# r9y9/deepvoice3_pytorch

Measured on AMD Instinct MI355X. Metric: mel-frames/sec/node (train step, deepvoice3_ljspeech), higher is better.
Workload: dtype f16x3

## Files before the change

deepvoice3_pytorch_amd/csrc/conv_gemm_bf16x3.hip:

```cpp
#include "conv_common.h"
#include <math.h>
#include <type_traits>

typedef __bf16 bf16x8 __attribute__((ext_vector_type(8)));
typedef __bf16 bf16x2 __attribute__((ext_vector_type(2)));
typedef _Float16 f16x8 __attribute__((ext_vector_type(8)));
typedef _Float16 f16x2 __attribute__((ext_vector_type(2)));
typedef float f32x2 __attribute__((ext_vector_type(2)));

namespace {

constexpr int BKC = 32;
constexpr int KB = 4;
constexpr int HALO_MAX = 64;

__device__ __forceinline__ void split8(const float (&v)[8], bf16x8& hi, bf16x8& lo) {
#pragma unroll
  for (int i = 0; i < 8; i += 2) {
    const f32x2 f = {v[i], v[i + 1]};
    const bf16x2 h = __builtin_convertvector(f, bf16x2);
    const f32x2 r = f - __builtin_convertvector(h, f32x2);
    const bf16x2 l = __builtin_convertvector(r, bf16x2);
    hi[i] = h[0]; hi[i + 1] = h[1];
    lo[i] = l[0]; lo[i + 1] = l[1];
  }
}

template <bool F16>
__device__ __forceinline__ f32x16 mma16(const bf16x8& a, const bf16x8& b, const f32x16& c) {
  if constexpr (F16)
    return __builtin_amdgcn_mfma_f32_32x32x16_f16(__builtin_bit_cast(f16x8, a), __builtin_bit_cast(f16x8, b), c, 0, 0, 0);
  else
    return __builtin_amdgcn_mfma_f32_32x32x16_bf16(a, b, c, 0, 0, 0);
}

template <typename T>
__device__ __forceinline__ T ldg_off(const void* base, uint32_t byte_off) {
  return *reinterpret_cast<const T*>(reinterpret_cast<const char*>(base) + byte_off);
}

constexpr int STAMP_SLOTS = 192;
__device__ unsigned long long g_x3_stamps[8 * STAMP_SLOTS * 2];

template <int WM, int WN, int NI, bool MASK, int ABL = 0, int TERMS = 3, int MI = 1, bool PP = false, bool F16 = false, int DPJ = 0, int KS = 1, bool FG = false>
__global__ __launch_bounds__(WM* WN * 64 * KS) void conv_gemm_bf16x3_kernel(const ConvArgs args) {
  static_assert(!FG || (!MASK && !F16 && TERMS == 3 && ABL == 0 && DPJ == 0), "fused gate backward: the unmasked bf16-pair forms");
  static_assert(!F16 || TERMS == 3, "the fp16 form is the three-term split");
  static_assert(KS == 1 || (KS == 2 && !PP && DPJ == 0 && ABL == 0), "k-split: two groups on the in-phase loop");
  static_assert(DPJ == 0 || (DPJ == 1 || DPJ == 3), "deep prefetch: 1 or 3 taps");
  static_assert(DPJ == 0 || (!PP && MI == 1 && ABL == 0 && TERMS == 3), "deep prefetch: the in-phase three-term tiles");
  constexpr int DA = DPJ == 0 ? 1 : (DPJ == 1 ? (MASK ? 3 : 4) : 3);
  constexpr int DX = DPJ == 0 ? 1 : (DPJ == 1 ? (MASK ? 3 : 4) : 2);
  static_assert(!PP || (WM * WN == 8 && MI == 1 && (ABL == 0 || ABL >= 10)), "ping-pong: 8 waves, one row sub-tile per wave");
  constexpr int BM = WM * MI * 64, BMH = WM * MI * 32, BN = WN * NI * 32;
  constexpr int NT = WM * WN * 64;
  constexpr int AU = KB * BM / NT;
  constexpr int XI = (KB * (BN + (DPJ == 1 ? 0 : HALO_MAX)) + NT - 1) / NT;
  static_assert(KB * BM % NT == 0, "A panel must split evenly");
  const dv3_conv_desc& p = args.d;

  extern __shared__ __attribute__((aligned(16))) unsigned char smem_raw[];
  const int J = DPJ ? DPJ : p.J, dil = p.dil;
  const int BNH = BN + (J - 1) * dil;
  const int xbuf = 2 * KB * BNH;
  const int wave_all = __builtin_amdgcn_readfirstlane((int)threadIdx.x >> 6);
  const int grp = KS > 1 ? wave_all / (WM * WN) : 0;
  const int grp_units = 2 * 2 * KB * BM + 2 * xbuf;
  bf16x8* const As = reinterpret_cast<bf16x8*>(smem_raw) + grp * grp_units;
  bf16x8* const Xs = As + 2 * 2 * KB * BM;

  const int tid = (int)threadIdx.x - grp * NT;
  const int lane = tid & 63;
  const int wave = wave_all - grp * (WM * WN);
  const int wm = wave / WN, wn = wave % WN;
  const int l31 = lane & 31, lhi = lane >> 5;

  const int pid = dv3_xcd_remap(blockIdx.x, args.n_blocks);
  const int mt = pid % args.m_tiles;
  const int nt = pid / args.m_tiles;
  const int n0 = nt * BN;

  const bool gated = (p.mode == DV3_EPI_GLU || p.mode == DV3_EPI_HIGHWAY);
  int h0b, h1b, lim0, lim1;
  if (gated) {
    h0b = mt * BMH; h1b = p.a_half + mt * BMH; lim0 = p.a_half; lim1 = p.lda;
  } else {
    h0b = mt * BM; h1b = mt * BM + BMH; lim0 = lim1 = p.lda;
  }

  const int Cin = p.Cin, T = p.Tout, lda = p.lda, B = p.B;
  const int Ntot = B * T;
  const int k8_total = args.kp >> 3;
  const bf16x8* __restrict__ Wh = reinterpret_cast<const bf16x8*>(p.a_split);
  const int64_t plane = (int64_t)J * k8_total * lda;
  const uint32_t* __restrict__ xmask = p.xmask;
  const float xscale = F16 ? (float)(1 << DV3_F16_ACT_SHIFT) : 1.0f;
  const float dscale = p.drop_scale * xscale;
  const bool xpw = !MASK && !F16 && TERMS == 3 && p.x_pair != 0;

  uint32_t vbits = 0;
#pragma unroll
  for (int ni = 0; ni < NI; ++ni) {
    const int n = n0 + wn * (NI * 32) + ni * 32 + l31;
    const int bc = n / T, tc = n - bc * T;
    for (int j = 0; j < J; ++j) {
      const int ts = tc + j * dil - p.padL;
      if (n < Ntot && ts >= 0 && ts < T) vbits |= 1u << (j * NI + ni);
    }
  }
  uint32_t need = 0;
  for (int j = 0; j < J; ++j) {
    const uint32_t all = ((1u << NI) - 1u) << (j * NI);
    if (!__all((vbits & all) == all)) need |= 1u << j;
  }
  need = __builtin_amdgcn_readfirstlane(need);

  uint32_t xoff[XI];
  uint32_t xmo[MASK ? XI : 1];
  int xsh[MASK ? XI : 1];
  int xk8[XI];
  const int n_items = KB * BNH;
  const bool xbf = (TERMS == 1) && (p.io_bf16 & DV3_IO_IN_BF16);
  const uint32_t xsz = xbf ? 2u : 4u;
  const uint32_t x_rsb = (uint32_t)p.x_rs * xsz, m_rsb = (uint32_t)p.xmask_rs * 4u;
#pragma unroll
  for (int i = 0; i < XI; ++i) {
    const int idx = tid + i * NT;
    const int k8 = idx / BNH, q = idx - k8 * BNH;
    const int f = n0 - p.padL + q;
    int bf = 0, tf = 0;
    if (idx < n_items && f >= 0 && f < Ntot) {
      bf = f / T;
      tf = f - bf * T;
    }
    xk8[i] = k8 < KB ? k8 * 8 : 0;
    xoff[i] = ((uint32_t)bf * (uint32_t)p.x_bs + (uint32_t)tf) * xsz + (uint32_t)xk8[i] * x_rsb;
    if (MASK) {
      xmo[i] = ((uint32_t)(bf * Cin) * (uint32_t)p.xmask_rs + (uint32_t)(tf >> 5)) * 4u + (uint32_t)xk8[i] * m_rsb;
      xsh[i] = tf & 31;
    }
  }
  uint32_t aoff[AU];
#pragma unroll
  for (int u = 0; u < AU; ++u) {
    const int idx = tid + u * NT;
    const int col = idx % BM, k8 = idx / BM;
    const bool hi_half = col >= BMH;
    const int gcol = (hi_half ? h1b : h0b) + (col - (hi_half ? BMH : 0));
    aoff[u] = (uint32_t)(k8 * lda + (gcol < lda ? gcol : 0)) * 16u;
  }

  bf16x8 ra[DA][2][AU];
  float rx[DX][XI][8];
  uint32_t rm[MASK ? DX : 1][MASK ? XI : 1][8];

  const int nchunks_all = (Cin + BKC - 1) / BKC;
  const int nch_first = KS > 1 ? (nchunks_all + 1) / 2 : nchunks_all;
  const int c_base = grp * nch_first;
  const int nchunks = grp == 0 ? nch_first : nchunks_all - nch_first;

  auto load_A = [&](int chunk_l, int j, int slot = 0) {
    const int chunk = chunk_l + c_base;
    const bf16x8* srch = Wh + (int64_t)(j * k8_total + chunk * KB) * lda;
    const bf16x8* srcl = srch + plane;
#pragma unroll
    for (int u = 0; u < AU; ++u) {
      ra[slot][0][u] = ldg_off<bf16x8>(srch, aoff[u]);
      if (TERMS == 3) ra[slot][1][u] = ldg_off<bf16x8>(srcl, aoff[u]);
    }
  };
  auto write_A = [&](int buf, int slot = 0) {
    bf16x8* dst = As + buf * (2 * KB * BM);
#pragma unroll
    for (int u = 0; u < AU; ++u) {
      dst[tid + u * NT] = ra[slot][0][u];
      if (TERMS == 3) dst[KB * BM + tid + u * NT] = ra[slot][1][u];
    }
  };
  auto load_X = [&](int chunk_l, int slot = 0) {
    const int c0 = (chunk_l + c_base) * BKC;
    if (c0 + BKC <= Cin) {
      const char* xb = reinterpret_cast<const char*>(p.x) + (int64_t)c0 * x_rsb;
      const char* mb = reinterpret_cast<const char*>(xmask) + (int64_t)c0 * m_rsb;
      if (TERMS == 1 && xbf) {
#pragma unroll
        for (int e = 0; e < 8; ++e) {
#pragma unroll
          for (int i = 0; i < XI; ++i) {
            rx[slot][i][e] = __uint_as_float((uint32_t)ldg_off<uint16_t>(xb + (int64_t)e * x_rsb, xoff[i]) << 16);
            if (MASK) rm[slot][i][e] = ldg_off<uint32_t>(mb + (int64_t)e * m_rsb, xmo[i]);
          }
        }
      } else {
#pragma unroll
        for (int e = 0; e < 8; ++e) {
#pragma unroll
          for (int i = 0; i < XI; ++i) {
            rx[slot][i][e] = ldg_off<float>(xb + (int64_t)e * x_rsb, xoff[i]);
            if (MASK) rm[slot][i][e] = ldg_off<uint32_t>(mb + (int64_t)e * m_rsb, xmo[i]);
          }
        }
      }
    } else {
#pragma unroll
      for (int i = 0; i < XI; ++i) {
#pragma unroll
        for (int e = 0; e < 8; ++e) {
          const uint32_t dc = (uint32_t)(min(c0 + xk8[i] + e, Cin - 1) - xk8[i]);
          rx[slot][i][e] = xbf ? __uint_as_float((uint32_t)ldg_off<uint16_t>(p.x, xoff[i] + dc * x_rsb) << 16)
                         : ldg_off<float>(p.x, xoff[i] + dc * x_rsb);
          if (MASK) rm[slot][i][e] = ldg_off<uint32_t>(xmask, xmo[MASK ? i : 0] + dc * m_rsb);
        }
      }
    }
  };
  auto write_X = [&](int buf, int slot = 0) {
    bf16x8* dst = Xs + buf * xbuf;
#pragma unroll
    for (int i = 0; i < XI; ++i) {
      const int idx = tid + i * NT;
      if (idx < n_items) {
        float v[8];
#pragma unroll
        for (int e = 0; e < 8; ++e) {
          v[e] = rx[slot][i][e];
          if (MASK) v[e] *= ((rm[slot][i][e] >> xsh[i]) & 1u) ? dscale : 0.f;
          else if (F16) v[e] *= xscale;
        }
        bf16x8 hi, lo;
        if constexpr (F16) dv3_note_range(args.range_ctr, dv3_split8_f16(v, hi, lo));
        else if constexpr (!MASK && TERMS == 3) {
          if (xpw) {
            uint32_t w[8];
#pragma unroll
            for (int e = 0; e < 8; ++e) w[e] = __float_as_uint(rx[slot][i][e]);
            dv3_pair_units(w, hi, lo);
          } else split8(v, hi, lo);
        } else split8(v, hi, lo);
        dst[idx] = hi;
        if (TERMS == 3) dst[KB * BNH + idx] = lo;
      }
    }
  };

  f32x16 acc[MI][2][NI];
#pragma unroll
  for (int mi = 0; mi < MI; ++mi)
#pragma unroll
    for (int h = 0; h < 2; ++h)
#pragma unroll
      for (int ni = 0; ni < NI; ++ni)
#pragma unroll
        for (int r = 0; r < 16; ++r) acc[mi][h][ni][r] = 0.f;

  const int nsteps = (ABL == 5 || ABL == 9) ? 0 : nchunks * J;
  const int a_off = wm * (MI * 32) + l31;
  const int x_off = wn * (NI * 32) + l31;

  if constexpr (DPJ == 0) {
    load_A(0, 0);
    load_X(0);
    write_A(0);
    write_X(0);
    __syncthreads();
  }

  int n_stamp = 0;
  auto stamp = [&]() {
    if constexpr (ABL == 10) {
      if (blockIdx.x == gridDim.x / 2 && n_stamp < STAMP_SLOTS) {
        const unsigned long long t0 = __builtin_amdgcn_s_memrealtime(), t1 = __builtin_readcyclecounter();
        if (lane == 0) {
          g_x3_stamps[(wave * STAMP_SLOTS + n_stamp) * 2] = t0;
          g_x3_stamps[(wave * STAMP_SLOTS + n_stamp) * 2 + 1] = t1;
        }
      }
      ++n_stamp;
    }
  };
  int c = 0, j = 0;
  if constexpr (PP) {
    const int late = wave >> 2;
    load_A((1 < nsteps && J == 1) ? 1 : 0, (1 < nsteps && J > 1) ? 1 : 0);
    if (1 < nchunks) load_X(1);
    stamp();
    const int prio = args.prio;
    if (prio == 3 && late) __builtin_amdgcn_s_setprio(1);
    if (prio == 4 && !late) __builtin_amdgcn_s_setprio(1);
    if (late) __syncthreads();
    for (int step = 0; step < nsteps; ++step) {
      const int cur = step & 1;
      int jn = j + 1, cn = c;
      if (jn == J) { jn = 0; cn = c + 1; }
      const bool has_next = step + 1 < nsteps;
      const bool new_chunk = has_next && jn == 0;
      stamp();
      if (prio == 1) __builtin_amdgcn_s_setprio(3);
      bf16x8 ah[2][2], al[2][2], bh[2][NI], bl[2][NI];
      {
        const bf16x8* AsH = As + cur * (2 * KB * BM);
        const bf16x8* AsL = AsH + KB * BM;
        const bf16x8* XsH = Xs + (c & 1) * xbuf;
        const bf16x8* XsL = XsH + KB * BNH;
        const bool fix = (need >> j) & 1u;
        const bf16x8 zero8 = {0, 0, 0, 0, 0, 0, 0, 0};
#pragma unroll
        for (int s = 0; s < 2; ++s) {
          const int k8 = 2 * s + lhi;
          const int ai = k8 * BM + a_off;
          ah[s][0] = AsH[ai];
          ah[s][1] = AsH[ai + BMH];
          al[s][0] = (TERMS == 3) ? AsL[ai] : ah[s][0];
          al[s][1] = (TERMS == 3) ? AsL[ai + BMH] : ah[s][1];
          const int xi = k8 * BNH + x_off + j * dil;
#pragma unroll
          for (int ni = 0; ni < NI; ++ni) {
            bh[s][ni] = XsH[xi + ni * 32];
            bl[s][ni] = (TERMS == 3) ? XsL[xi + ni * 32] : bh[s][ni];
          }
        }
        if (fix) {
#pragma unroll
          for (int s = 0; s < 2; ++s)
#pragma unroll
            for (int ni = 0; ni < NI; ++ni) {
              const bool ok = (vbits >> (j * NI + ni)) & 1u;
              bh[s][ni] = ok ? bh[s][ni] : zero8;
              if (TERMS == 3) bl[s][ni] = ok ? bl[s][ni] : zero8;
            }
        }
      }
      stamp();
      write_A(cur ^ 1);
      stamp();
      if (new_chunk) {
        write_X((c + 1) & 1);
        if (cn + 1 < nchunks) load_X(cn + 1);
      }
      {
        int j2 = jn + 1, c2 = cn;
        if (j2 == J) { j2 = 0; c2 = cn + 1; }
        const bool more = step + 2 < nsteps;
        load_A(more ? c2 : c, more ? j2 : j);
      }
      stamp();
      __syncthreads();
      stamp();
      if (prio == 1) __builtin_amdgcn_s_setprio(0);
      if (prio == 2) __builtin_amdgcn_s_setprio(3);
#pragma unroll
      for (int s = 0; s < 2; ++s) {
        if (TERMS == 3) {
#pragma unroll
          for (int ni = 0; ni < NI; ++ni) {
            acc[0][0][ni] = mma16<F16>(al[s][0], bh[s][ni], acc[0][0][ni]);
            acc[0][1][ni] = mma16<F16>(al[s][1], bh[s][ni], acc[0][1][ni]);
          }
#pragma unroll
          for (int ni = 0; ni < NI; ++ni) {
            acc[0][0][ni] = mma16<F16>(ah[s][0], bl[s][ni], acc[0][0][ni]);
            acc[0][1][ni] = mma16<F16>(ah[s][1], bl[s][ni], acc[0][1][ni]);
          }
        }
#pragma unroll
        for (int ni = 0; ni < NI; ++ni) {
          acc[0][0][ni] = mma16<F16>(ah[s][0], bh[s][ni], acc[0][0][ni]);
          acc[0][1][ni] = mma16<F16>(ah[s][1], bh[s][ni], acc[0][1][ni]);
        }
      }
      stamp();
      if (prio == 2) __builtin_amdgcn_s_setprio(0);
      if (has_next || !late) __syncthreads();
      j = jn;
      c = cn;
    }
    stamp();
  } else if constexpr (DPJ > 0) {
    constexpr int U = (DPJ == 1 && DA == 4) ? 4 : 6;
    static_assert(U % DA == 0 && (U / DPJ) % DX == 0 && U % DPJ == 0 && U % 2 == 0 && (U / DPJ) % 2 == 0,
                  "ring slots and LDS buffer parities must be compile-time");
    const int last_step = nsteps - 1, last_chunk = nchunks - 1;
#pragma unroll
    for (int a = 0; a < DA; ++a)
#pragma unroll
      for (int u = 0; u < AU; ++u) ra[a][0][u] = ra[a][1][u] = bf16x8{0, 0, 0, 0, 0, 0, 0, 0};
#pragma unroll
    for (int x = 0; x < DX; ++x)
#pragma unroll
      for (int i = 0; i < XI; ++i)
#pragma unroll
        for (int e = 0; e < 8; ++e) {
          rx[x][i][e] = 0.f;
          if (MASK) rm[x][i][e] = 0u;
        }
    int s_first = -U;
    asm volatile("" : "+s"(s_first));
    for (int s0 = s_first; s0 < nsteps; s0 += U) {
#pragma unroll
      for (int dd = 0; dd < U; ++dd) {
        const int s = s0 + dd;
        const int jj = dd % DPJ;
        const int cx = dd / DPJ;
        {
          const int sa = min(max(s + DA, 0), last_step);
          load_A(sa / DPJ, sa % DPJ, dd % DA);
        }
        if (jj == 0) load_X(min(max(s0 / DPJ + cx + DX, 0), last_chunk), cx % DX);
        if (s >= 0 && s < nsteps) {
          const bf16x8* AsH = As + (dd & 1) * (2 * KB * BM);
          const bf16x8* AsL = AsH + KB * BM;
          const bf16x8* XsH = Xs + (cx & 1) * xbuf;
          const bf16x8* XsL = XsH + KB * BNH;
          const bool fix = (need >> jj) & 1u;
          const bf16x8 zero8 = {0, 0, 0, 0, 0, 0, 0, 0};
#pragma unroll
          for (int s2 = 0; s2 < 2; ++s2) {
            const int k8 = 2 * s2 + lhi;
            const int ai = k8 * BM + a_off;
            const bf16x8 ah0 = AsH[ai], ah1 = AsH[ai + BMH], al0 = AsL[ai], al1 = AsL[ai + BMH];
            bf16x8 bh[NI], bl[NI];
            const int xi = k8 * BNH + x_off + jj * dil;
#pragma unroll
            for (int ni = 0; ni < NI; ++ni) {
              bh[ni] = XsH[xi + ni * 32];
              bl[ni] = XsL[xi + ni * 32];
            }
            if (fix) {
#pragma unroll
              for (int ni = 0; ni < NI; ++ni) {
                const bool ok = (vbits >> (jj * NI + ni)) & 1u;
                bh[ni] = ok ? bh[ni] : zero8;
                bl[ni] = ok ? bl[ni] : zero8;
              }
            }
#pragma unroll
            for (int ni = 0; ni < NI; ++ni) {
              acc[0][0][ni] = mma16<F16>(al0, bh[ni], acc[0][0][ni]);
              acc[0][1][ni] = mma16<F16>(al1, bh[ni], acc[0][1][ni]);
            }
#pragma unroll
            for (int ni = 0; ni < NI; ++ni) {
              acc[0][0][ni] = mma16<F16>(ah0, bl[ni], acc[0][0][ni]);
              acc[0][1][ni] = mma16<F16>(ah1, bl[ni], acc[0][1][ni]);
            }
#pragma unroll
            for (int ni = 0; ni < NI; ++ni) {
              acc[0][0][ni] = mma16<F16>(ah0, bh[ni], acc[0][0][ni]);
              acc[0][1][ni] = mma16<F16>(ah1, bh[ni], acc[0][1][ni]);
            }
          }
        }
        write_A((dd & 1) ^ 1, (dd + 1) % DA);
        if (jj == DPJ - 1) write_X((cx & 1) ^ 1, (cx + 1) % DX);
        __syncthreads();
      }
    }
  } else
  for (int step = 0; step < (KS > 1 ? nch_first * J : nsteps); ++step) {
    if (KS > 1 && step >= nsteps) {
      __syncthreads();
      continue;
    }
    const int cur = step & 1;
    int jn = j + 1, cn = c;
    if (jn == J) { jn = 0; cn = c + 1; }
    const bool has_next = step + 1 < nsteps;
    const bool new_chunk = has_next && jn == 0;
    if (ABL != 1 && ABL != 2 && ABL != 3) {
      if (has_next) load_A(cn, jn);
      if (j == 0 && c + 1 < nchunks) load_X(c + 1);
    }

    {
      const bf16x8* AsH = As + cur * (2 * KB * BM);
      const bf16x8* AsL = AsH + KB * BM;
      const bf16x8* XsH = Xs + (c & 1) * xbuf;
      const bf16x8* XsL = XsH + KB * BNH;
      const bool fix = (need >> j) & 1u;
      const bf16x8 zero8 = {0, 0, 0, 0, 0, 0, 0, 0};
#pragma unroll
      for (int s = 0; s < 2; ++s) {
        const int k8 = 2 * s + lhi;
        const int ai = k8 * BM + a_off;
        bf16x8 ah[MI][2], al[MI][2];
#pragma unroll
        for (int mi = 0; mi < MI; ++mi) {
          ah[mi][0] = AsH[ai + mi * 32];
          ah[mi][1] = AsH[ai + mi * 32 + BMH];
          al[mi][0] = ah[mi][0];
          al[mi][1] = ah[mi][1];
          if (TERMS == 3) { al[mi][0] = AsL[ai + mi * 32]; al[mi][1] = AsL[ai + mi * 32 + BMH]; }
        }
        bf16x8 bh[NI], bl[NI];
        const int xi = k8 * BNH + x_off + j * dil;
#pragma unroll
        for (int ni = 0; ni < NI; ++ni) {
          bh[ni] = XsH[xi + ni * 32];
          bl[ni] = (TERMS == 3) ? XsL[xi + ni * 32] : bh[ni];
        }
        if (fix) {
#pragma unroll
          for (int ni = 0; ni < NI; ++ni) {
            const bool ok = (vbits >> (j * NI + ni)) & 1u;
            bh[ni] = ok ? bh[ni] : zero8;
            if (TERMS == 3) bl[ni] = ok ? bl[ni] : zero8;
          }
        }
        if (ABL == 4) {
#pragma unroll
          for (int mi = 0; mi < MI; ++mi) asm volatile("" ::"v"(ah[mi][0]), "v"(ah[mi][1]), "v"(al[mi][0]), "v"(al[mi][1]));
#pragma unroll
          for (int ni = 0; ni < NI; ++ni) asm volatile("" ::"v"(bh[ni]), "v"(bl[ni]));
          continue;
        }
        if (TERMS == 3) {
#pragma unroll
          for (int mi = 0; mi < MI; ++mi)
#pragma unroll
            for (int ni = 0; ni < NI; ++ni) {
              acc[mi][0][ni] = mma16<F16>(al[mi][0], bh[ni], acc[mi][0][ni]);
              acc[mi][1][ni] = mma16<F16>(al[mi][1], bh[ni], acc[mi][1][ni]);
            }
#pragma unroll
          for (int mi = 0; mi < MI; ++mi)
#pragma unroll
            for (int ni = 0; ni < NI; ++ni) {
              acc[mi][0][ni] = mma16<F16>(ah[mi][0], bl[ni], acc[mi][0][ni]);
              acc[mi][1][ni] = mma16<F16>(ah[mi][1], bl[ni], acc[mi][1][ni]);
            }
        }
#pragma unroll
        for (int mi = 0; mi < MI; ++mi)
#pragma unroll
          for (int ni = 0; ni < NI; ++ni) {
            acc[mi][0][ni] = mma16<F16>(ah[mi][0], bh[ni], acc[mi][0][ni]);
            acc[mi][1][ni] = mma16<F16>(ah[mi][1], bh[ni], acc[mi][1][ni]);
          }
      }
    }

    if (ABL != 2 && ABL != 3) {
      if (has_next) write_A(cur ^ 1);
      if (new_chunk) write_X((c + 1) & 1);
    }
    if (ABL != 3) __syncthreads();
    j = jn;
    c = cn;
  }

  if constexpr (KS > 1) {
    float* red = reinterpret_cast<float*>(reinterpret_cast<bf16x8*>(smem_raw) + grp_units);
    constexpr int NR = MI * 2 * NI * 16;
    static_assert((size_t)WM * WN * NR * 64 * 4 <= (size_t)(2 * 2 * KB * BM) * 16, "the accumulator image must fit one group's panels");
    float* mine = red + (wave * NR) * 64 + lane;
    if (grp == 1) {
#pragma unroll
      for (int mi = 0; mi < MI; ++mi)
#pragma unroll
        for (int h = 0; h < 2; ++h)
#pragma unroll
          for (int ni = 0; ni < NI; ++ni)
#pragma unroll
            for (int r = 0; r < 16; ++r) mine[(((mi * 2 + h) * NI + ni) * 16 + r) * 64] = acc[mi][h][ni][r];
    }
    __syncthreads();
    if (grp == 1) return;
#pragma unroll
    for (int mi = 0; mi < MI; ++mi)
#pragma unroll
      for (int h = 0; h < 2; ++h)
#pragma unroll
        for (int ni = 0; ni < NI; ++ni)
#pragma unroll
          for (int r = 0; r < 16; ++r) acc[mi][h][ni][r] += mine[(((mi * 2 + h) * NI + ni) * 16 + r) * 64];
  }
  if ((ABL != 6 && ABL != 9) || acc[0][0][0][0] + acc[MI - 1][1][0][0] + acc[0][0][NI - 1][5] + acc[MI - 1][1][NI - 1][7] == 1.2345e30f) {
    static_assert(MI == 1 || MI == 2, "row sub-tiles per wave");
    if constexpr (F16) {
      constexpr float kInv = 1.0f / (float)(1 << (DV3_F16_WEIGHT_SHIFT + DV3_F16_ACT_SHIFT));
#pragma unroll
      for (int mi = 0; mi < MI; ++mi)
#pragma unroll
        for (int h = 0; h < 2; ++h)
#pragma unroll
          for (int ni = 0; ni < NI; ++ni)
#pragma unroll
            for (int r = 0; r < 16; ++r) acc[mi][h][ni][r] *= kInv;
    }
    int n0e = n0;
    asm volatile("" : "+s"(n0e));
    int bcol[NI], tcol[NI];
    bool okc[NI];
#pragma unroll
    for (int ni = 0; ni < NI; ++ni) {
      const int n = n0e + wn * (NI * 32) + ni * 32 + l31;
      okc[ni] = n < Ntot;
      bcol[ni] = n / T;
      tcol[ni] = n - bcol[ni] * T;
    }
    if constexpr (FG) {
      const int nw0 = n0e + wn * (NI * 32);
      bool wide_done = false;
      if constexpr (NI == 2) {
        if (dv3_wide_gate_ok(p, args.wide) && (size_t)(WM * WN) * DV3_WIDE_LDS <= (size_t)(2 * 2 * KB * BM + 2 * xbuf) * 16) {
          float* wl = reinterpret_cast<float*>(smem_raw) + wave * (DV3_WIDE_LDS / 4);
#pragma unroll
          for (int mi = 0; mi < MI; ++mi) {
            const int row0 = wm * (MI * 32) + mi * 32;
            conv_epilogue_wide_block_gate<BM, BMH>(p, acc[mi][0], mt, row0, 0, lane, nw0, Ntot, wl);
            conv_epilogue_wide_block_gate<BM, BMH>(p, acc[mi][1], mt, row0, 1, lane, nw0, Ntot, wl);
          }
          wide_done = true;
        }
      }
      if (!wide_done) {
        conv_epilogue_dgrad_gate<BM, BMH, NI>(p, acc[0], mt, wm * (MI * 32), lhi, l31, bcol, tcol, okc, nw0 >> 5);
        if (MI == 2) conv_epilogue_dgrad_gate<BM, BMH, NI>(p, acc[MI - 1], mt, wm * (MI * 32) + 32, lhi, l31, bcol, tcol, okc, nw0 >> 5);
      }
    } else
    if (TERMS == 1 && (p.io_bf16 & DV3_IO_OUT_C8)) {
      conv_epilogue_c8<BM, BMH, NI>(p, acc[0], gated, mt, wm * (MI * 32), lhi, bcol, tcol, okc);
      if (MI == 2) conv_epilogue_c8<BM, BMH, NI>(p, acc[MI - 1], gated, mt, wm * (MI * 32) + 32, lhi, bcol, tcol, okc);
    } else if (NI == 2 && TERMS == 3 && ABL == 0 && dv3_wide_epilogue_ok(p, args.wide) &&
               (size_t)(WM * WN) * DV3_WIDE_LDS <= (size_t)(2 * 2 * KB * BM + 2 * xbuf) * 16) {
      if constexpr (NI == 2) {
        float* wl = reinterpret_cast<float*>(smem_raw) + wave * (DV3_WIDE_LDS / 4);
        const int nw0 = n0e + wn * (NI * 32);
#pragma unroll
        for (int mi = 0; mi < MI; ++mi) {
          const int row0 = wm * (MI * 32) + mi * 32;
          conv_epilogue_wide_block<BM, BMH>(p, acc[mi][0], mt, row0, 0, lane, nw0, Ntot, wl);
          conv_epilogue_wide_block<BM, BMH>(p, acc[mi][1], mt, row0, 1, lane, nw0, Ntot, wl);
        }
      }
    } else {
      conv_epilogue<BM, BMH, NI, ABL, TERMS == 1>(p, acc[0], gated, mt, wm * (MI * 32), lhi, bcol, tcol, okc);
      if (MI == 2)
        conv_epilogue<BM, BMH, NI, ABL, TERMS == 1>(p, acc[MI - 1], gated, mt, wm * (MI * 32) + 32, lhi, bcol, tcol, okc);
    }
  }
  stamp();
}

__global__ __launch_bounds__(256) void split_pack_kernel(const float* __restrict__ src,
                                                         bf16x8* __restrict__ dst, int J, int K,
                                                         int lda, int k8_total, int dtype, uint32_t* range_ctr) {
  const int64_t n = (int64_t)J * k8_total * lda;
  const int64_t idx = (int64_t)blockIdx.x * 256 + threadIdx.x;
  if (idx >= n) return;
  const int m = (int)(idx % lda);
  const int64_t row = idx / lda;
  const int j = (int)(row / k8_total), k8 = (int)(row % k8_total);
  float v[8];
#pragma unroll
  for (int i = 0; i < 8; ++i) {
    const int k = k8 * 8 + i;
    v[i] = (k < K) ? src[((int64_t)j * K + k) * lda + m] : 0.f;
    if (dtype == DV3_SPLIT_DTYPE_F16) v[i] *= (float)(1 << DV3_F16_WEIGHT_SHIFT);
  }
  bf16x8 hi, lo;
  if (dtype == DV3_SPLIT_DTYPE_F16) dv3_note_range(range_ctr, dv3_split8_f16(v, hi, lo)); else split8(v, hi, lo);
  dst[idx] = hi;
  dst[n + idx] = lo;
}

#ifdef DV3_X3_ISA_ONLY
#ifndef DV3_X3_ISA_KS
#define DV3_X3_ISA_KS 1
#endif
template __global__ void conv_gemm_bf16x3_kernel<2, 2, 1, DV3_X3_ISA_MASK, 0, 3, 1, false, DV3_X3_ISA_F16, DV3_X3_ISA_DPJ, DV3_X3_ISA_KS>(const ConvArgs);
}
#else
template <int WM, int WN, int NI, bool MASK, int TERMS, int MI = 1, bool PP = false, bool F16 = false, int DPJ = 0, int KS = 1, bool FG = false>
int launch_x3_m(const ConvArgs& a, size_t lds, hipStream_t st) {
  static bool attr_set = false;
  if (!attr_set) {
    hipError_t e = hipFuncSetAttribute((const void*)conv_gemm_bf16x3_kernel<WM, WN, NI, MASK, 0, TERMS, MI, PP, F16, DPJ, KS, FG>,
                                       hipFuncAttributeMaxDynamicSharedMemorySize, 160 * 1024);
    if (e != hipSuccess) {
      dv3_set_error("conv_gemm_bf16x3: hipFuncSetAttribute: %s", hipGetErrorString(e));
      return DV3_ELAUNCH;
    }
    attr_set = true;
  }
  dim3 grid(a.n_blocks), block(WM * WN * 64 * KS);
  hipLaunchKernelGGL((conv_gemm_bf16x3_kernel<WM, WN, NI, MASK, 0, TERMS, MI, PP, F16, DPJ, KS, FG>), grid, block, lds * KS, st, a);
  return dv3_check_launch("conv_gemm_bf16x3");
}
int g_x3_ablate = 0;
#ifdef DV3_EXPERIMENTS
template <int ABL>
int launch_x3_abl(const ConvArgs& a, size_t lds, hipStream_t st) {
  (void)hipFuncSetAttribute((const void*)conv_gemm_bf16x3_kernel<2, 2, 2, false, ABL>,
                      hipFuncAttributeMaxDynamicSharedMemorySize, 160 * 1024);
  hipLaunchKernelGGL((conv_gemm_bf16x3_kernel<2, 2, 2, false, ABL>), dim3(a.n_blocks), dim3(256), lds, st, a);
  return dv3_check_launch("conv_gemm_bf16x3(abl)");
}
#endif
int g_x3_pingpong = 1;
template <int WM, int WN, int NI, int MI, bool PP>
int launch_x3_big_pp(const ConvArgs& a, size_t lds, hipStream_t st) {
  if (a.d.split_terms == DV3_SPLIT_F16X3)
    return a.d.xmask ? launch_x3_m<WM, WN, NI, true, 3, MI, PP, true>(a, lds, st) : launch_x3_m<WM, WN, NI, false, 3, MI, PP, true>(a, lds, st);
  if (a.d.split_terms == 1)
    return a.d.xmask ? launch_x3_m<WM, WN, NI, true, 1, MI, PP>(a, lds, st) : launch_x3_m<WM, WN, NI, false, 1, MI, PP>(a, lds, st);
  return a.d.xmask ? launch_x3_m<WM, WN, NI, true, 3, MI, PP>(a, lds, st) : launch_x3_m<WM, WN, NI, false, 3, MI, PP>(a, lds, st);
}
template <int WM, int WN, int NI, int MI>
int launch_x3_big(const ConvArgs& a, size_t lds, hipStream_t st) {
#ifdef DV3_EXPERIMENTS
  if constexpr (WM == 2 && WN == 4 && MI == 1) {
    if (g_x3_ablate == 10 && g_x3_pingpong && !a.d.xmask && (a.d.split_terms == 0 || a.d.split_terms == 3)) {
      (void)hipFuncSetAttribute((const void*)conv_gemm_bf16x3_kernel<2, 4, 2, false, 10, 3, 1, true>,
                                hipFuncAttributeMaxDynamicSharedMemorySize, 160 * 1024);
      hipLaunchKernelGGL((conv_gemm_bf16x3_kernel<2, 4, 2, false, 10, 3, 1, true>), dim3(a.n_blocks), dim3(512), lds, st, a);
      return dv3_check_launch("conv_gemm_bf16x3(stamps)");
    }
  }
#endif
  if constexpr (WM * WN == 8 && MI == 1) {
    if (g_x3_pingpong) return launch_x3_big_pp<WM, WN, NI, MI, true>(a, lds, st);
  }
  return launch_x3_big_pp<WM, WN, NI, MI, false>(a, lds, st);
}
template <int WM, int WN, int NI>
int launch_x3(const ConvArgs& a, size_t lds, hipStream_t st) {
#ifdef DV3_EXPERIMENTS
  if (g_x3_ablate && WM == 2 && WN == 2 && NI == 2 && !a.d.xmask && (a.d.split_terms == 0 || a.d.split_terms == 3)) {
    switch (g_x3_ablate) {
      case 1: return launch_x3_abl<1>(a, lds, st);
      case 2: return launch_x3_abl<2>(a, lds, st);
      case 3: return launch_x3_abl<3>(a, lds, st);
      case 4: return launch_x3_abl<4>(a, lds, st);
      case 5: return launch_x3_abl<5>(a, lds, st);
      case 6: return launch_x3_abl<6>(a, lds, st);
      case 7: return launch_x3_abl<7>(a, lds, st);
      case 8: return launch_x3_abl<8>(a, lds, st);
      case 9: return launch_x3_abl<9>(a, lds, st);
    }
  }
#endif
  if constexpr (WM == 2 && WN == 2 && NI == 1) {
    if (a.ks == 2 && a.d.split_terms != 1) {
      const bool f16 = a.d.split_terms == DV3_SPLIT_F16X3, m = a.d.xmask != nullptr;
      if (f16) return m ? launch_x3_m<2, 2, 1, true, 3, 1, false, true, 0, 2>(a, lds, st) : launch_x3_m<2, 2, 1, false, 3, 1, false, true, 0, 2>(a, lds, st);
      return m ? launch_x3_m<2, 2, 1, true, 3, 1, false, false, 0, 2>(a, lds, st) : launch_x3_m<2, 2, 1, false, 3, 1, false, false, 0, 2>(a, lds, st);
    }
  }
#ifdef DV3_EXPERIMENTS
  if constexpr (WM == 2 && WN == 2 && NI == 1) {
    if (a.dp == 1 || a.dp == 3) {
      const bool f16 = a.d.split_terms == DV3_SPLIT_F16X3, m = a.d.xmask != nullptr;
      if (a.dp == 1) {
        if (f16) return m ? launch_x3_m<2, 2, 1, true, 3, 1, false, true, 1>(a, lds, st) : launch_x3_m<2, 2, 1, false, 3, 1, false, true, 1>(a, lds, st);
        return m ? launch_x3_m<2, 2, 1, true, 3, 1, false, false, 1>(a, lds, st) : launch_x3_m<2, 2, 1, false, 3, 1, false, false, 1>(a, lds, st);
      }
      if (f16) return m ? launch_x3_m<2, 2, 1, true, 3, 1, false, true, 3>(a, lds, st) : launch_x3_m<2, 2, 1, false, 3, 1, false, true, 3>(a, lds, st);
      return m ? launch_x3_m<2, 2, 1, true, 3, 1, false, false, 3>(a, lds, st) : launch_x3_m<2, 2, 1, false, 3, 1, false, false, 3>(a, lds, st);
    }
  }
#endif
  if (a.d.split_terms == DV3_SPLIT_F16X3)
    return a.d.xmask ? launch_x3_m<WM, WN, NI, true, 3, 1, false, true>(a, lds, st) : launch_x3_m<WM, WN, NI, false, 3, 1, false, true>(a, lds, st);
  if (a.d.split_terms == 1)
    return a.d.xmask ? launch_x3_m<WM, WN, NI, true, 1>(a, lds, st) : launch_x3_m<WM, WN, NI, false, 1>(a, lds, st);
  return a.d.xmask ? launch_x3_m<WM, WN, NI, true, 3>(a, lds, st) : launch_x3_m<WM, WN, NI, false, 3>(a, lds, st);
}

int g_x3_ks = 1;
int g_x3_ks_max_blocks = 256, g_x3_ks_min_steps = 8;
int g_x3_dp = 0;
int g_x3_rel8 = 86;
int g_x3_j1_flat = 1;
int g_x3_rel2 = 112;
const TileCfg* pick_tile_x3(const dv3_conv_desc* d, bool gated, int want_tile) {
  const TileCfg* best = nullptr;
  double best_cost = 0;
  const int64_t ntot = (int64_t)d->B * d->Tout;
  for (const TileCfg& c : kCfgs) {
    if (want_tile && c.id != want_tile) continue;
    if (d->pg && !(c.id == 1 || c.id == 2 || c.id == 8 || c.id == 9)) continue;
    const int BM = c.wm * c.mi * 64, BMH = c.wm * c.mi * 32, BN = c.wn * c.ni * 32;
    const int64_t mt = gated ? dv3_cdiv(d->Cg, BMH) : dv3_cdiv(d->M, BM);
    const int64_t ntl = dv3_cdiv64(ntot, BN);
    const double slots = c.id > 6 ? 256.0 : 512.0;
    const double blocks = (double)mt * ntl;
    const double full = floor(blocks / slots), rem = blocks - slots * full;
    const double rounds = (full + (rem == 0 ? 0.0 : (c.id <= 6 && rem <= 256 ? 0.6 : 1.0))) * (slots / 512.0);
    static const double kRel[10] = {0, 1.0, 1.12, 2.0, 2.2, 1.8, 2.0, 9.9, 0.93, 0.87};
    double rel = c.id == 2 ? g_x3_rel2 * 0.01 : c.id == 8 ? g_x3_rel8 * 0.01 : kRel[c.id];
    if (g_x3_j1_flat && d->J == 1 && d->Cin <= 512 && (c.id == 1 || c.id == 2 || c.id == 8 || c.id == 9)) rel = 1.0;
    const double cost = rounds * BM * BN * rel;
    if (!best || cost < best_cost) {
      best = &c;
      best_cost = cost;
    }
  }
  return best;
}

}

int g_x3_pp2 = 128;
extern int g_pp2_ord, g_pp2_ord_u, g_pp2_ord_m, g_pp2_abl, g_pp2_sk, g_pp2_sk_overhead, g_pp2_sk_gain, g_pp2_sk_abl, g_pp2_fast_tail;
int g_x3_pp2_sk_units = 8;
int dv3_conv_gemm_pp2_dispatch(const dv3_conv_desc* d, hipStream_t st);
int g_x3_wide = 1;
int g_x3_prio = 0;

int dv3_conv_gemm_bf16x3_dispatch(const dv3_conv_desc* d, hipStream_t st) {
  const bool gated = d->mode == DV3_EPI_GLU || d->mode == DV3_EPI_HIGHWAY;
  if (d->a_bs != 0 || (d->lda & 3) || d->Tin != d->Tout) return 1;
  if ((d->J - 1) * d->dil > HALO_MAX || d->J * 2 > 32) return 1;
  if ((int64_t)d->B * d->Tout >= (1ll << 30) || (int64_t)d->B * d->x_bs >= (1ll << 30)) return 1;
  if (d->xmask && (int64_t)d->B * d->Cin * d->xmask_rs >= (1ll << 30)) return 1;
  if ((int64_t)d->J * ((d->Cin + 31) / 32 * 4) * d->lda >= (1ll << 27)) return 1;
  const bool gated0 = d->mode == DV3_EPI_GLU || d->mode == DV3_EPI_HIGHWAY;
  const int64_t pp2_tiles = (int64_t)(gated0 ? dv3_cdiv(d->Cg, 128) : dv3_cdiv(d->M, 256)) * dv3_cdiv64((int64_t)d->B * d->Tout, 256);
  const bool sk_fill = d->sk_ws && g_pp2_sk && (d->mode != DV3_EPI_DGRAD || g_pp2_sk >= 2) && g_x3_pp2 > 0 && pp2_tiles * (d->Cin / 32) >= (int64_t)g_x3_pp2_sk_units * 256;
  if (d->tile_hint == 30 || (g_x3_pp2 > 0 && d->tile_hint == 0 && (pp2_tiles >= g_x3_pp2 || sk_fill))) {
    const int rc = dv3_conv_gemm_pp2_dispatch(d, st);
    if (rc != 1) return rc;
    if (d->tile_hint == 30) return 1;
  }
  const TileCfg* best = pick_tile_x3(d, gated, d->tile_hint > 20 ? d->tile_hint - 20 : 0);
  if (!best) return 1;
  bool ks_ok = false;
  if (g_x3_ks && d->split_terms != 1 && (d->tile_hint == 0 || d->tile_hint == 22)) {
    const int64_t nb2 = (int64_t)(gated ? dv3_cdiv(d->Cg, 64) : dv3_cdiv(d->M, 128)) * dv3_cdiv64((int64_t)d->B * d->Tout, 64);
    const int nch = (d->Cin + 31) / 32;
    const int ksteps = nch * d->J;
    ks_ok = nch >= 2 && (g_x3_ks == 2 || (ksteps >= g_x3_ks_min_steps && nb2 <= (ksteps >= 16 ? g_x3_ks_max_blocks : g_x3_ks_max_blocks * 5 / 8)));
    if (ks_ok && d->tile_hint == 0 && (best->id == 4 || best->id == 6)) best = &kCfgs[1];
  }
  const int BM = best->wm * best->mi * 64, BMH = best->wm * best->mi * 32, BN = best->wn * best->ni * 32;
  const int BNH = BN + (d->J - 1) * d->dil;
  const size_t lds = (size_t)(2 * 2 * KB * BM + 2 * 2 * KB * BNH) * 16;
  if (lds > 160 * 1024) return 1;
  ConvArgs a;
  a.d = *d;
  a.a_scalar = 0;
  a.wide = g_x3_wide;
  a.prio = g_x3_prio;
  a.range_ctr = d->split_terms == DV3_SPLIT_F16X3 ? dv3_range_ctr() : nullptr;
  a.kp = (d->Cin + 31) / 32 * 32;
  a.m_tiles = gated ? dv3_cdiv(d->Cg, BMH) : dv3_cdiv(d->M, BM);
  a.n_tiles = (int)dv3_cdiv64((int64_t)d->B * d->Tout, BN);
  const int64_t nb = (int64_t)a.m_tiles * a.n_tiles;
  DV3_REQUIRE(nb < (1ll << 31), "conv_gemm: grid too large");
  a.n_blocks = (int)nb;
  a.ks = (ks_ok && best->id == 2 && 2 * lds <= 160 * 1024) ? 2 : 0;
  a.dp = 0;
#ifdef DV3_EXPERIMENTS
  if (best->id == 2 && d->split_terms != 1 && (d->J == 1 || d->J == 3) && g_x3_dp) {
    if (g_x3_dp == 2 || nb <= 2 * 256) a.dp = d->J;
  }
#endif
  g_dv3_last_conv = (d->split_terms == 1 ? 4000 : d->split_terms == DV3_SPLIT_F16X3 ? 5000 : 3000) + best->id * 10 +
                    ((best->id >= 8 && g_x3_pingpong) ? 1 : 0) + (a.dp ? 5 : 0) + (a.ks == 2 ? 2 : 0);
  if (d->pg) {
    if (d->xmask || d->split_terms == DV3_SPLIT_F16X3 || d->split_terms == 1) return 1;
    g_dv3_last_conv += 600;
    switch (best->id) {
      case 1: return launch_x3_m<2, 2, 2, false, 3, 1, false, false, 0, 1, true>(a, lds, st);
      case 2: return a.ks == 2 ? launch_x3_m<2, 2, 1, false, 3, 1, false, false, 0, 2, true>(a, lds, st)
                               : launch_x3_m<2, 2, 1, false, 3, 1, false, false, 0, 1, true>(a, lds, st);
      case 8: return launch_x3_m<4, 2, 2, false, 3, 1, true, false, 0, 1, true>(a, lds, st);
      case 9: return launch_x3_m<2, 4, 2, false, 3, 1, true, false, 0, 1, true>(a, lds, st);
    }
    return 1;
  }
  switch (best->id) {
    case 1: return launch_x3<2, 2, 2>(a, lds, st);
    case 2: return launch_x3<2, 2, 1>(a, lds, st);
    case 3: return launch_x3<4, 1, 1>(a, lds, st);
    case 4: return launch_x3<2, 1, 1>(a, lds, st);
    case 5: return launch_x3<1, 2, 2>(a, lds, st);
    case 6: return launch_x3<1, 2, 1>(a, lds, st);
    case 7: return launch_x3_big<2, 2, 2, 2>(a, lds, st);
    case 8: return launch_x3_big<4, 2, 2, 1>(a, lds, st);
    case 9: return launch_x3_big<2, 4, 2, 1>(a, lds, st);
  }
  return 1;
}

extern int g_wgrad_tile, g_wgrad_prio, g_wgrad_t2_abl, g_wgrad_taps2_default, g_wgrad_t2_window, g_wgrad_t2_il;
extern int g_spk_prefetch;
extern int g_gate_c8_fast;
extern int g_loss_fast_log;
extern int g_gate_vec;
extern int g_wn_bwd_vec4;
extern int g_wgrad_c8_pf2, g_wgrad_c8_il, g_wgrad_c8_tr, g_spk_abl;
int dv3_planes_debug_set(int what, int value);
int dv3_c8pp_debug_set(int what, int value);
int dv3_conv_census_set(int on);
extern "C" int dv3_debug_set(int what, int value) {
#ifndef DV3_EXPERIMENTS
  DV3_REQUIRE(!(value != 0 && (what == 1 || what == 6 || what == 13 || what == 16 || what == 21 || what == 26 || what == 28 || what == 32 || what == 43)),
              "debug_set(%d, %d): ablation variants are not in this build (make EXP=1)", what, value);
#endif
  if (what >= 4 && what <= 8) return dv3_planes_debug_set(what, value);
  if (what == 40) return dv3_conv_census_set(value);
  if (what == 19 || what == 21 || what == 30 || what == 32 || (what >= 34 && what <= 36)) return dv3_c8pp_debug_set(what, value);
  if (what == 20) g_wgrad_c8_pf2 = value;
  if (what == 49) g_wgrad_c8_il = value;
  if (what == 9) g_x3_rel2 = value;
  if (what == 12) g_x3_pp2 = value;
  if (what == 13) g_pp2_abl = value;
  if (what == 29 || what == 31) {
    const bool ship = value == 0 || value == 17 || value == 81;
#ifndef DV3_EXPERIMENTS
    DV3_REQUIRE(ship, "debug_set(%d, %d): this LOAD-phase variant is not in this build (make EXP=1)", what, value);
#endif
    if (what == 29) { g_pp2_ord_u = ship ? value : 0; g_pp2_ord = ship ? 0 : value; }
    else g_pp2_ord_m = ship ? value : 0;
  }
  if (what == 50) g_pp2_fast_tail = value;
  if (what == 51) g_wn_bwd_vec4 = value;
  if (what == 52) g_wgrad_c8_tr = value;
  if (what == 54) g_spk_prefetch = value;
  if (what == 55) g_gate_vec = value;
  if (what == 56) g_gate_c8_fast = value;
  if (what == 57) g_loss_fast_log = value;
  if (what == 22) g_pp2_sk = value;
  if (what == 23) g_pp2_sk_overhead = value;
  if (what == 24) g_pp2_sk_gain = value;
  if (what == 25) g_x3_pp2_sk_units = value;
  if (what == 26) g_pp2_sk_abl = value;
  if (what == 27) g_x3_j1_flat = value;
  if (what == 43) g_x3_dp = value;
  if (what == 42) g_x3_rel8 = value;
  if (what == 44) g_x3_ks = value;
  if (what == 45) g_x3_ks_max_blocks = value;
  if (what == 46) g_x3_ks_min_steps = value;
  if (what == 28) g_spk_abl = value;
  if (what == 14) g_x3_prio = value;
  if (what == 18) g_x3_wide = value;
  if (what == 15) g_wgrad_prio = value;
  if (what == 16) g_wgrad_t2_abl = value;
  if (what == 17) g_wgrad_taps2_default = value;
  if (what == 47) g_wgrad_t2_window = value;
  if (what == 48) g_wgrad_t2_il = value;
  if (what == 1) g_x3_ablate = value;
  if (what == 2) g_wgrad_tile = value;
  if (what == 3) g_x3_pingpong = value;
  return DV3_OK;
}

int dv3_pp2_read_stamps(void* dst, int64_t bytes);
int dv3_decode_read_stamps(void* dst, int64_t bytes);
int dv3_conv_census_read(int what, void* dst, int64_t bytes);
extern "C" int dv3_debug_read(int what, void* dst, int64_t bytes) {
  if (what == 40 || what == 41) return dv3_conv_census_read(what, dst, bytes);
  if (what == 2 && dst) return dv3_pp2_read_stamps(dst, bytes);
  if (what == 3 && dst) return dv3_decode_read_stamps(dst, bytes);
  DV3_REQUIRE(what == 1 && dst && bytes > 0 && bytes <= (int64_t)sizeof(unsigned long long) * 8 * STAMP_SLOTS * 2,
              "debug_read: bad arguments");
  hipError_t e = hipMemcpyFromSymbol(dst, HIP_SYMBOL(g_x3_stamps), (size_t)bytes, 0, hipMemcpyDeviceToHost);
  if (e != hipSuccess) {
    dv3_set_error("debug_read: %s", hipGetErrorString(e));
    return DV3_ELAUNCH;
  }
  return DV3_OK;
}

extern "C" int dv3_split_pack_bf16(const float* packed, uint16_t* out, int32_t J, int32_t K,
                                   int32_t lda, int32_t dtype, void* stream) {
  DV3_REQUIRE(dtype == DV3_SPLIT_DTYPE_BF16 || dtype == DV3_SPLIT_DTYPE_F16, "split_pack: bad dtype");
  DV3_REQUIRE(packed && out, "split_pack: null pointer");
  DV3_REQUIRE(J >= 1 && K >= 1 && lda >= 1 && ((uintptr_t)out & 15) == 0, "split_pack: bad arguments");
  const int k8_total = (K + 31) / 32 * 4;
  const int64_t n = (int64_t)J * k8_total * lda;
  hipLaunchKernelGGL(split_pack_kernel, dim3((unsigned)dv3_cdiv64(n, 256)), dim3(256), 0,
                     (hipStream_t)stream, packed, reinterpret_cast<bf16x8*>(out), J, K, lda, k8_total, (int)dtype,
                     dv3_range_ctr());
  return dv3_check_launch("split_pack_bf16");
}
#endif
```

deepvoice3_pytorch_amd/csrc/conv_gemm_pp2.hip:

```cpp
#include "conv_common.h"
#include <math.h>
#include <type_traits>

typedef __bf16 bf16x8 __attribute__((ext_vector_type(8)));
typedef __bf16 bf16x2 __attribute__((ext_vector_type(2)));
typedef _Float16 f16x8 __attribute__((ext_vector_type(8)));
typedef float f32x2 __attribute__((ext_vector_type(2)));

namespace {

constexpr int BKC = 32, KB = 4, HALO_MAX = 64;
constexpr int BM = 256, BMH = 128, BN = 256, NT = 512, MI = 2, NI = 2, WN = 4;
constexpr int JT = 3;
constexpr int AU = KB * BM / NT;
constexpr int XI = (KB * (BN + HALO_MAX) + NT - 1) / NT;
static_assert(AU == 2, "one panel unit per k16 phase");

__device__ __forceinline__ void pp2_split8(const float (&v)[8], bf16x8& hi, bf16x8& lo) {
#pragma unroll
  for (int i = 0; i < 8; i += 2) {
    const f32x2 f = {v[i], v[i + 1]};
    const bf16x2 h = __builtin_convertvector(f, bf16x2);
    const f32x2 r = f - __builtin_convertvector(h, f32x2);
    const bf16x2 l = __builtin_convertvector(r, bf16x2);
    hi[i] = h[0]; hi[i + 1] = h[1];
    lo[i] = l[0]; lo[i + 1] = l[1];
  }
}
template <bool F16>
__device__ __forceinline__ f32x16 pp2_mma(const bf16x8& a, const bf16x8& b, const f32x16& c) {
  if constexpr (F16)
    return __builtin_amdgcn_mfma_f32_32x32x16_f16(__builtin_bit_cast(f16x8, a), __builtin_bit_cast(f16x8, b), c, 0, 0, 0);
  else
    return __builtin_amdgcn_mfma_f32_32x32x16_bf16(a, b, c, 0, 0, 0);
}
template <bool OPAQUE>
__device__ __forceinline__ const ConvArgs* dv3_opaque_args(const ConvArgs* a) {
  if constexpr (OPAQUE) {
    int off = 0;
    asm volatile("" : "+s"(off));
    return reinterpret_cast<const ConvArgs*>(reinterpret_cast<const char*>(a) + off);
  } else {
    return a;
  }
}
template <typename T>
__device__ __forceinline__ T pp2_ldg(const void* base, uint32_t byte_off) {
  return *reinterpret_cast<const T*>(reinterpret_cast<const char*>(base) + byte_off);
}

constexpr int PP2_STAMPS = 320;
__device__ unsigned long long g_pp2_stamps[8 * PP2_STAMPS * 2];

template <bool MASK, bool F16, int ABL = 0, bool SK = false, int ORD = 0, bool PW = false, bool FG = false>
__global__ __launch_bounds__(NT) void conv_gemm_pp2_kernel(const ConvArgs args) {
  static_assert(!PW || (!MASK && !F16 && !SK), "pair words: the unmasked bf16-pair tile-per-workgroup form");
  static_assert(!FG || (!MASK && !F16 && !SK), "fused gate backward: the unmasked bf16-pair tile-per-workgroup form");
  const dv3_conv_desc& p = args.d;
  int n_stamp = 0;
  auto stamp = [&]() {
    if constexpr (ABL == 4) {
      if (blockIdx.x == gridDim.x / 2 + 3 && n_stamp < PP2_STAMPS) {
        const unsigned long long t0 = __builtin_amdgcn_s_memrealtime(), t1 = __builtin_readcyclecounter();
        if ((threadIdx.x & 63) == 0) {
          g_pp2_stamps[((threadIdx.x >> 6) * PP2_STAMPS + n_stamp) * 2] = t0;
          g_pp2_stamps[((threadIdx.x >> 6) * PP2_STAMPS + n_stamp) * 2 + 1] = t1;
        }
      }
      ++n_stamp;
    }
  };
  stamp();
  extern __shared__ __attribute__((aligned(16))) unsigned char smem_raw[];
  constexpr int J = JT;
  bf16x8* const As = reinterpret_cast<bf16x8*>(smem_raw);
  bf16x8* const Xs = As + 2 * 2 * KB * BM;

  int pid_ = dv3_xcd_remap(blockIdx.x, args.n_blocks);
  if constexpr (SK) {
    const int q = 1 << args.sk_qshift;
    pid_ = (pid_ & ~(q - 1)) + (q - 1 - (pid_ & (q - 1)));
  }
  const int pid = pid_;
  const int nchunks = p.Cin / BKC;
  int seg_u = 0, seg_end = 0, sk_base = 0, sk_rem = 0, sk_g0 = 0;
  if constexpr (SK) {
    const int grp = pid >> args.sk_qshift, slot = pid & ((1 << args.sk_qshift) - 1);
    const bool big = grp < args.sk_tr;
    sk_base = big ? args.sk_base : args.sk_base2;
    sk_rem = big ? args.sk_rem : args.sk_rem2;
    sk_g0 = (grp * args.sk_tg + min(grp, args.sk_tr)) << args.sk_shift;
    seg_u = sk_g0 + slot * sk_base + min(slot, sk_rem);
    seg_end = seg_u + sk_base + (slot < sk_rem ? 1 : 0);
  }
  constexpr bool DMA_A = ABL == 11;
  constexpr bool WIDE_GLU = (ORD & 32) != 0;
  int tid_ = threadIdx.x;
  const int wave_s = __builtin_amdgcn_readfirstlane(tid_ >> 6);
  do {
  const ConvArgs& A = *dv3_opaque_args<SK>(&args);
  const dv3_conv_desc& p = A.d;
  const int dil = p.dil;
  const int BNH = BN + (J - 1) * dil;
  const int xbuf = 2 * KB * BNH;
  if constexpr (SK) {
    int lane_;
    asm volatile("v_mbcnt_lo_u32_b32 %0, -1, 0\n\tv_mbcnt_hi_u32_b32 %0, -1, %0" : "=v"(lane_));
    tid_ = wave_s * 64 + lane_;
  }
  const int tid = tid_;
  const int lane = tid & 63;
  const int wave = __builtin_amdgcn_readfirstlane(tid >> 6);
  const int wm = wave / WN, wn = wave % WN;
  const int l31 = lane & 31, lhi = lane >> 5;
  int tile_ = pid, c0_ = 0, c1_ = nchunks;
  if constexpr (SK) {
    tile_ = seg_u >> A.sk_shift;
    c0_ = seg_u - tile_ * nchunks;
    c1_ = min(nchunks, c0_ + (seg_end - seg_u));
  }
  const int tile = tile_, c0 = SK ? c0_ : 0, c1 = SK ? c1_ : nchunks;
  const int mt = SK ? (tile & (A.m_tiles - 1)) : tile % A.m_tiles;
  const int nt = SK ? (tile >> A.sk_mshift) : tile / A.m_tiles;
  const int n0 = nt * BN;

  const bool gated = (p.mode == DV3_EPI_GLU || p.mode == DV3_EPI_HIGHWAY);
  int h0b, h1b;
  if (gated) {
    h0b = mt * BMH; h1b = p.a_half + mt * BMH;
  } else {
    h0b = mt * BM; h1b = mt * BM + BMH;
  }

  const int Cin = p.Cin, T = p.Tout, lda = p.lda, B = p.B;
  const int Ntot = B * T;
  const int k8_total = A.kp >> 3;
  const bf16x8* __restrict__ Wh = reinterpret_cast<const bf16x8*>(p.a_split);
  const int64_t plane = (int64_t)J * k8_total * lda;
  const float xscale = F16 ? (float)(1 << DV3_F16_ACT_SHIFT) : 1.0f;
  const float dscale = p.drop_scale * xscale;

  uint32_t vbits = 0;
#pragma unroll
  for (int ni = 0; ni < NI; ++ni) {
    const int n = n0 + wn * (NI * 32) + ni * 32 + l31;
    const int bc = n / T, tc = n - bc * T;
    for (int j = 0; j < J; ++j) {
      const int ts = tc + j * dil - p.padL;
      if (n < Ntot && ts >= 0 && ts < T) vbits |= 1u << (j * NI + ni);
    }
  }
  uint32_t need = 0;
  for (int j = 0; j < J; ++j) {
    const uint32_t all = ((1u << NI) - 1u) << (j * NI);
    if (!__all((vbits & all) == all)) need |= 1u << j;
  }
  need = __builtin_amdgcn_readfirstlane(need);

  uint32_t xoff[XI];
  const int n_items = KB * BNH;
  const uint32_t x_rsb = (uint32_t)p.x_rs * 4u;
  const uint32_t c8p = (uint32_t)((Cin + 31) / 32 * 4);
#pragma unroll
  for (int i = 0; i < XI; ++i) {
    const int idx = tid + i * NT;
    const int k8 = idx / BNH, q = idx - k8 * BNH;
    const int f = n0 - p.padL + q;
    int bf = 0, tf = 0;
    if (idx < n_items && f >= 0 && f < Ntot) {
      bf = f / T;
      tf = f - bf * T;
    }
    const int xk8 = k8 < KB ? k8 * 8 : 0;
    xoff[i] = ((uint32_t)bf * (uint32_t)p.x_bs + (uint32_t)tf) * 4u + (uint32_t)xk8 * x_rsb;
  }
  constexpr bool LEAN = (ORD & 2) != 0 && !SK;
  uint32_t aoff_r[2] = {0u, 0u};
  auto aoff_of = [&](int u) -> uint32_t {
    if constexpr (LEAN) return aoff_r[u];
    int t_ = tid;
    asm volatile("" : "+v"(t_));
    const int idx = t_ + u * NT;
    const int col = idx % BM, k8 = idx / BM;
    const bool hi_half = col >= BMH;
    const int gcol = (hi_half ? h1b : h0b) + (col - (hi_half ? BMH : 0));
    return (uint32_t)(k8 * lda + (gcol < lda ? gcol : 0)) * 16u;
  };

  if constexpr (LEAN) {
#pragma unroll
    for (int u = 0; u < 2; ++u) {
      const int idx = tid + u * NT;
      const int col = idx % BM, k8 = idx / BM;
      const bool hi_half = col >= BMH;
      const int gcol = (hi_half ? h1b : h0b) + (col - (hi_half ? BMH : 0));
      aoff_r[u] = (uint32_t)(k8 * lda + (gcol < lda ? gcol : 0)) * 16u;
    }
  }

  bf16x8 ra[2];
  float rx[XI][8];
  uint32_t rk[MASK ? XI : 1];

  auto load_A_unit = [&](int chunk, int j, auto uc) {
    constexpr int u = decltype(uc)::value;
    const bf16x8* srch = Wh + (int64_t)(j * k8_total + chunk * KB) * lda;
    const uint32_t ao = aoff_of(u);
    ra[0] = pp2_ldg<bf16x8>(srch, ao);
    ra[1] = pp2_ldg<bf16x8>(srch + plane, ao);
  };
  auto write_A_unit = [&](int buf, auto uc) {
    constexpr int u = decltype(uc)::value;
    bf16x8* dst = As + buf * (2 * KB * BM);
    dst[tid + u * NT] = ra[0];
    dst[KB * BM + tid + u * NT] = ra[1];
  };
  auto dma_A_unit = [&](int buf, int chunk, int j, auto uc) {
    constexpr int u = decltype(uc)::value;
    const bf16x8* srch = Wh + (int64_t)(j * k8_total + chunk * KB) * lda;
    const uint32_t ao = aoff_of(u);
    bf16x8* dst = As + buf * (2 * KB * BM) + u * NT + wave * 64;
    typedef const __attribute__((address_space(1))) void* gptr;
    typedef __attribute__((address_space(3))) void* lptr;
    __builtin_amdgcn_global_load_lds((gptr)(reinterpret_cast<const char*>(srch) + ao), (lptr)dst, 16, 0, 0);
    __builtin_amdgcn_global_load_lds((gptr)(reinterpret_cast<const char*>(srch + plane) + ao), (lptr)(dst + KB * BM), 16, 0, 0);
  };
  auto load_X_half = [&](int chunk, auto ic, auto hc) {
    constexpr int i = decltype(ic)::value, h = decltype(hc)::value;
    const char* xb = reinterpret_cast<const char*>(p.x) + (int64_t)(chunk * BKC) * x_rsb;
    uint32_t rs = x_rsb;
    asm volatile("" : "+s"(rs));
#pragma unroll
    for (int e = 4 * h; e < 4 * h + 4; ++e) {
      uint32_t er = (uint32_t)e * rs;
      if constexpr (SK) {
        if (e == 0) { er = 0; asm volatile("" : "+s"(er)); }
      }
      rx[i][e] = pp2_ldg<float>(xb, xoff[i] + er);
    }
    if constexpr (MASK && h == 1) {
      int t_ = tid;
      asm volatile("" : "+v"(t_));
      const int idx = t_ + i * NT;
      const int k8 = idx / BNH, q = idx - k8 * BNH;
      const int f = n0 - p.padL + q;
      int bf = 0, tf = 0;
      if (idx < n_items && f >= 0 && f < Ntot) {
        bf = f / T;
        tf = f - bf * T;
      }
      const uint32_t mo = ((uint32_t)bf * c8p + (uint32_t)(k8 < KB ? k8 : 0)) * (uint32_t)T + (uint32_t)tf;
      rk[i] = (uint32_t)pp2_ldg<uint8_t>(p.xmask_c8 + (int64_t)chunk * 4 * T, mo);
    }
  };
  auto write_X_item = [&](int buf, auto ic) {
    constexpr int i = decltype(ic)::value;
    bf16x8* dst = Xs + buf * xbuf;
    const int idx = tid + i * NT;
    float v[8];
    uint32_t keep = MASK ? rk[i] : 0u;
    if constexpr (MASK && SK) asm("" : "+v"(keep));
#pragma unroll
    for (int e = 0; e < 8; ++e) {
      v[e] = rx[i][e];
      if constexpr (MASK) v[e] *= ((keep >> e) & 1u) ? dscale : 0.f;
      else if (F16) v[e] *= xscale;
    }
    bf16x8 hi, lo;
    if constexpr (PW) {
      uint32_t w[8];
#pragma unroll
      for (int e = 0; e < 8; ++e) w[e] = __float_as_uint(rx[i][e]);
      dv3_pair_units(w, hi, lo);
    } else if constexpr (F16 && LEAN) {
      const float m0 = fmaxf(fmaxf(fabsf(v[0]), fabsf(v[1])), fabsf(v[2]));
      const float m1 = fmaxf(fmaxf(fabsf(v[3]), fabsf(v[4])), fabsf(v[5]));
      const float m = fmaxf(fmaxf(m0, m1), fmaxf(fabsf(v[6]), fabsf(v[7])));
      const bool bad = !(m <= 65504.f);
      if (__builtin_expect(__any(bad), 0)) {
        dv3_note_range(A.range_ctr, dv3_split8_f16(v, hi, lo));
      } else {
        f16x8 h8, l8;
#pragma unroll
        for (int e = 0; e < 8; e += 2) {
          const f32x2 f = {v[e], v[e + 1]};
          typedef _Float16 f16x2_ __attribute__((ext_vector_type(2)));
          const f16x2_ h = __builtin_convertvector(f, f16x2_);
          h8[e] = h[0]; h8[e + 1] = h[1];
          if constexpr ((ORD & 8) != 0) {
            uint32_t l2 = 0u;
            const uint32_t h2 = __builtin_bit_cast(uint32_t, h);
            asm("v_fma_mixlo_f16 %0, %1, -1.0, %2 op_sel:[0,0,0] op_sel_hi:[1,0,0]" : "+v"(l2) : "v"(h2), "v"(v[e]));
            asm("v_fma_mixhi_f16 %0, %1, -1.0, %2 op_sel:[1,0,0] op_sel_hi:[1,0,0]" : "+v"(l2) : "v"(h2), "v"(v[e + 1]));
            const f16x2_ l = __builtin_bit_cast(f16x2_, l2);
            l8[e] = l[0]; l8[e + 1] = l[1];
          } else {
            l8[e] = (_Float16)(v[e] - (float)h[0]);
            l8[e + 1] = (_Float16)(v[e + 1] - (float)h[1]);
          }
        }
        hi = __builtin_bit_cast(bf16x8, h8);
        lo = __builtin_bit_cast(bf16x8, l8);
      }
    } else if constexpr (F16) dv3_note_range(A.range_ctr, dv3_split8_f16(v, hi, lo)); else pp2_split8(v, hi, lo);
    if (idx < n_items) {
      dst[idx] = hi;
      dst[KB * BNH + idx] = lo;
    }
  };
  uint32_t sbad = 0;
  auto write_X_item_nb = [&](int buf, auto ic) {
    constexpr int i = decltype(ic)::value;
    bf16x8* dst = Xs + buf * xbuf;
    const int idx = tid + i * NT;
    float v[8];
    const uint32_t keep = MASK ? rk[i] : 0u;
#pragma unroll
    for (int e = 0; e < 8; ++e) {
      v[e] = rx[i][e];
      if constexpr (MASK) {
        v[e] *= ((keep >> e) & 1u) ? dscale : 0.f;
        asm("" : "+v"(v[e]));
      } else if (F16) v[e] *= xscale;
    }
    bf16x8 hi, lo;
    if constexpr (PW) {
      uint32_t w[8];
#pragma unroll
      for (int e = 0; e < 8; ++e) w[e] = __float_as_uint(rx[i][e]);
      dv3_pair_units(w, hi, lo);
    } else if constexpr (F16) {
      const bool bad = dv3_split8_f16(v, hi, lo);
      sbad += (uint32_t)__builtin_popcountll(__ballot(bad));
    } else {
      pp2_split8(v, hi, lo);
    }
    const int spare = 2 * xbuf - buf * xbuf;
    const bool live = i < 2 || idx < n_items;
    dst[live ? idx : spare] = hi;
    dst[live ? KB * BNH + idx : spare + 1] = lo;
  };
  using U0 = std::integral_constant<int, 0>;
  using U1 = std::integral_constant<int, 1>;
  using U2 = std::integral_constant<int, 2>;
  constexpr bool CVC = (ORD & 64) != 0 && !SK;
  static_assert(XI == 3 && JT == 3, "three activation items per thread, one per tap's pair of k16 phases");

  f32x16 acc[MI][2][NI];
  float zero_ = 0.f;
  if constexpr (SK) asm volatile("" : "+v"(zero_));
#pragma unroll
  for (int mi = 0; mi < MI; ++mi)
#pragma unroll
    for (int h = 0; h < 2; ++h)
#pragma unroll
      for (int ni = 0; ni < NI; ++ni)
#pragma unroll
        for (int r = 0; r < 16; ++r) acc[mi][h][ni][r] = zero_;

  const int a_off = wm * (MI * 32) + l31;
  const int x_off = wn * (NI * 32) + l31;

  load_A_unit(c0, 0, U0{});
  write_A_unit(0, U0{});
  load_A_unit(c0, 0, U1{});
  load_X_half(c0, U0{}, U0{}); load_X_half(c0, U0{}, U1{});
  load_X_half(c0, U1{}, U0{}); load_X_half(c0, U1{}, U1{});
  load_X_half(c0, U2{}, U0{}); load_X_half(c0, U2{}, U1{});
  write_A_unit(0, U1{});
  write_X_item(0, U0{});
  write_X_item(0, U1{});
  write_X_item(0, U2{});
  __syncthreads();
  {
    const int cp = min(c0 + 1, c1 - 1);
    if (!DMA_A) load_A_unit(c0, 1, U0{});
    load_X_half(cp, U0{}, U0{});
    load_X_half(cp, U0{}, U1{});
    load_X_half(cp, U1{}, U0{}); load_X_half(cp, U1{}, U1{});
    load_X_half(cp, U2{}, U0{});
    if constexpr (!CVC) load_X_half(cp, U2{}, U1{});
  }

  const bool pf_on = (ORD & 4) != 0 && !SK && gated && p.r != nullptr;
  const int late = wave >> 2;
  stamp();
  if (late) __syncthreads();
  for (int c = c0; c < c1; ++c) {
    const int cr = c - c0;
    const bf16x8* XsH = Xs + (cr & 1) * xbuf;
    const bf16x8* XsL = XsH + KB * BNH;
    const int cx = min(c + 2, c1 - 1);
    const bool last_chunk = c + 1 == c1;
#pragma unroll
    for (int q = 0; q < 2 * JT; ++q) {
      constexpr int dummy = 0; (void)dummy;
      const int j = q >> 1, s = q & 1;
      const int cur = (cr * JT + j) & 1;
      const bf16x8* AsH = As + cur * (2 * KB * BM);
      const bf16x8* AsL = AsH + KB * BM;
      const bool fix = (need >> j) & 1u;
      stamp();
      bf16x8 ah[MI][2], al[MI][2], bh[NI], bl[NI];
      auto read_frags = [&](bool do_a, bool do_b) {
        const int k8 = 2 * s + lhi;
        if (do_a) {
          const int ai = k8 * BM + a_off;
#pragma unroll
          for (int mi = 0; mi < MI; ++mi) {
            ah[mi][0] = AsH[ai + mi * 32];
            ah[mi][1] = AsH[ai + mi * 32 + BMH];
            al[mi][0] = AsL[ai + mi * 32];
            al[mi][1] = AsL[ai + mi * 32 + BMH];
          }
        }
        if (do_b) {
          const int xi = k8 * BNH + x_off + j * dil;
#pragma unroll
          for (int ni = 0; ni < NI; ++ni) {
            bh[ni] = XsH[xi + ni * 32];
            bl[ni] = XsL[xi + ni * 32];
          }
        }
      };
      auto fix_frags = [&]() {
        const int k8 = 2 * s + lhi; (void)k8;
        if (fix) {
          const bf16x8 zero8 = {0, 0, 0, 0, 0, 0, 0, 0};
#pragma unroll
          for (int ni = 0; ni < NI; ++ni) {
            const bool ok = (vbits >> (j * NI + ni)) & 1u;
            bh[ni] = ok ? bh[ni] : zero8;
            bl[ni] = ok ? bl[ni] : zero8;
          }
        }
      };
      if constexpr ((ORD & 1) != 0) {
        read_frags(true, (ORD & 16) == 0);
        __builtin_amdgcn_sched_barrier(0);
      }
      if (ABL != 2) {
        int jn = j + 1, cn = c;
        if (jn >= JT) { jn = 0; cn = c + 1; }
        int j2 = jn + 1, c2 = cn;
        if (j2 >= JT) { j2 = 0; c2 = cn + 1; }
        if (cn >= c1) { cn = c; jn = j; }
        if (c2 >= c1) { c2 = c; j2 = j; }
        if constexpr (DMA_A) {
          if (s == 0) {
            dma_A_unit(cur ^ 1, cn, jn, U0{});
            dma_A_unit(cur ^ 1, cn, jn, U1{});
          }
          (void)c2; (void)j2;
        } else if (s == 0) {
          if (ABL != 9) write_A_unit(cur ^ 1, U0{});
          if (ABL != 7) load_A_unit(cn, jn, U1{});
        } else {
          if (ABL != 9) write_A_unit(cur ^ 1, U1{});
          if (ABL != 7) load_A_unit(c2, j2, U0{});
        }
        constexpr bool WX = ABL != 8, LX = ABL != 6;
        if constexpr (CVC) {
          const int cx1 = min(c + 1, c1 - 1);
          if (q == 0) load_X_half(cx1, U2{}, U1{});
          if (q == 1) load_X_half(cx, U0{}, U0{});
          if (q == 2) load_X_half(cx, U0{}, U1{});
          if (q == 3) load_X_half(cx, U1{}, U0{});
          if (q == 4) load_X_half(cx, U1{}, U1{});
          if (q == 5) load_X_half(cx, U2{}, U0{});
        } else {
        if (q == 0) { if (WX) write_X_item((cr + 1) & 1, U0{}); if (LX) load_X_half(cx, U0{}, U0{}); }
        if (q == 1) { if (LX) load_X_half(cx, U0{}, U1{}); }
        if (q == 2) { if (WX) write_X_item((cr + 1) & 1, U1{}); if (LX) load_X_half(cx, U1{}, U0{}); }
        if (q == 3) { if (LX) load_X_half(cx, U1{}, U1{}); }
        if (q == 4) { if (WX) write_X_item((cr + 1) & 1, U2{}); if (LX) load_X_half(cx, U2{}, U0{}); }
        if (q == 5) { if (LX) load_X_half(cx, U2{}, U1{}); }
        }
        if constexpr ((ORD & 4) != 0 && !SK) {
          if ((q == 1 || q == 3) && last_chunk && pf_on) {
            typedef const __attribute__((address_space(1))) void* gptr;
            typedef __attribute__((address_space(3))) void* lptr;
            unsigned char* strip = smem_raw + (size_t)(2 * 2 * KB * BM + 2 * xbuf) * 16 + wave * 256;
            int t_ = tid;
            asm volatile("" : "+v"(t_));
            const int row = t_ >> 2, col = (t_ & 3) * 64 + (q >> 1) * 32;
            const int ch = min(mt * BMH + row, p.Cg - 1);
            const int n = min(n0 + col, Ntot - 1);
            const int bb = n / T, tt = n - bb * T;
            const uint32_t po = ((uint32_t)bb * (uint32_t)p.r_bs + (uint32_t)ch * (uint32_t)p.r_rs + (uint32_t)tt) * 4u;
            __builtin_amdgcn_global_load_lds((gptr)(reinterpret_cast<const char*>(p.r) + po), (lptr)strip, 4, 0, 0);
          }
        }
      }
      __builtin_amdgcn_sched_barrier(0);
      stamp();
      if constexpr ((ORD & 1) == 0) read_frags(true, true);
      else if constexpr ((ORD & 16) != 0) read_frags(false, true);
      fix_frags();
      if constexpr (ABL == 4) {
        asm volatile("s_waitcnt lgkmcnt(0)" ::: "memory");
        stamp();
      }
      __syncthreads();
      if (ABL != 5) __builtin_amdgcn_sched_barrier(0);
      stamp();
      if (ABL != 1) {
#pragma unroll
        for (int mi = 0; mi < MI; ++mi)
#pragma unroll
          for (int ni = 0; ni < NI; ++ni) {
            acc[mi][0][ni] = pp2_mma<F16>(al[mi][0], bh[ni], acc[mi][0][ni]);
            acc[mi][1][ni] = pp2_mma<F16>(al[mi][1], bh[ni], acc[mi][1][ni]);
          }
#pragma unroll
        for (int mi = 0; mi < MI; ++mi)
#pragma unroll
          for (int ni = 0; ni < NI; ++ni) {
            acc[mi][0][ni] = pp2_mma<F16>(ah[mi][0], bl[ni], acc[mi][0][ni]);
            acc[mi][1][ni] = pp2_mma<F16>(ah[mi][1], bl[ni], acc[mi][1][ni]);
          }
#pragma unroll
        for (int mi = 0; mi < MI; ++mi)
#pragma unroll
          for (int ni = 0; ni < NI; ++ni) {
            acc[mi][0][ni] = pp2_mma<F16>(ah[mi][0], bh[ni], acc[mi][0][ni]);
            acc[mi][1][ni] = pp2_mma<F16>(ah[mi][1], bh[ni], acc[mi][1][ni]);
          }
      } else {
#pragma unroll
        for (int mi = 0; mi < MI; ++mi) asm volatile("" ::"v"(ah[mi][0]), "v"(ah[mi][1]), "v"(al[mi][0]), "v"(al[mi][1]));
#pragma unroll
        for (int ni = 0; ni < NI; ++ni) asm volatile("" ::"v"(bh[ni]), "v"(bl[ni]));
      }
      if constexpr (CVC) {
        if (q == 0) write_X_item_nb((cr + 1) & 1, U0{});
        if (q == 2) write_X_item_nb((cr + 1) & 1, U1{});
        if (q == 4) write_X_item_nb((cr + 1) & 1, U2{});
        if ((q & 1) == 0) {
#pragma unroll
          for (int m = 0; m < 22; ++m) {
            __builtin_amdgcn_sched_group_barrier(0x008, 1, 0);
            __builtin_amdgcn_sched_group_barrier(0x002, 3, 0);
          }
          __builtin_amdgcn_sched_group_barrier(0x008, 1, 0);
          __builtin_amdgcn_sched_group_barrier(0x200, 1, 0);
          __builtin_amdgcn_sched_group_barrier(0x008, 1, 0);
          __builtin_amdgcn_sched_group_barrier(0x200, 1, 0);
        }
      }
      stamp();
      if (ABL != 5) __builtin_amdgcn_sched_barrier(0);
      if (!(last_chunk && q == 2 * JT - 1) || !late) __syncthreads();
    }
  }
  stamp();
  if constexpr (CVC && F16) {
    if (sbad != 0 && lane == 0 && A.range_ctr) atomicAdd(A.range_ctr, sbad);
  }

  bool run_tail = true;
  if constexpr (SK) {
    constexpr int ACC = MI * 2 * NI * 16;
#ifdef DV3_EXPERIMENTS
    const int sk_abl = A.sk_abl;
#else
    constexpr int sk_abl = 0;
#endif
    float* const ws = A.sk_ws;
    int* const flags = A.sk_flags;
    if (c0 != 0) {
      char* dst = reinterpret_cast<char*>(ws) + ((size_t)pid * (ACC * NT) + (size_t)tid * 4) * 4;
      if (!(sk_abl & 1))
#pragma unroll
      for (int mi = 0; mi < MI; ++mi)
#pragma unroll
        for (int h = 0; h < 2; ++h)
#pragma unroll
          for (int ni = 0; ni < NI; ++ni)
#pragma unroll
            for (int r4 = 0; r4 < 4; ++r4) {
              typedef float f32x4_ __attribute__((ext_vector_type(4)));
              const f32x4_ v4 = {acc[mi][h][ni][r4 * 4], acc[mi][h][ni][r4 * 4 + 1], acc[mi][h][ni][r4 * 4 + 2], acc[mi][h][ni][r4 * 4 + 3]};
              const char* d4 = dst + (size_t)((((mi * 2 + h) * NI + ni) * 4 + r4) * NT) * 16;
              asm volatile("global_store_dwordx4 %0, %1, off sc0 sc1" ::"v"(d4), "v"(v4) : "memory");
            }
      asm volatile("s_waitcnt vmcnt(0)" ::: "memory");
      __builtin_amdgcn_fence(__ATOMIC_RELEASE, "workgroup");
      __syncthreads();
      if (tid == 0) __hip_atomic_store(flags + pid, 1, __ATOMIC_RELAXED, __HIP_MEMORY_SCOPE_AGENT);
      run_tail = false;
    } else if (c1 < nchunks) {
      const int qm = (1 << A.sk_qshift) - 1;
      for (int w2 = pid + 1; (w2 & qm) != 0; ++w2) {
        const int s2 = sk_g0 + (w2 & qm) * sk_base + min(w2 & qm, sk_rem);
        if (s2 >= (tile + 1) * nchunks) break;
        if (tid == 0 && !(sk_abl & 4))
          while (__hip_atomic_load(flags + w2, __ATOMIC_RELAXED, __HIP_MEMORY_SCOPE_AGENT) == 0) __builtin_amdgcn_s_sleep(8);
        __syncthreads();
        __builtin_amdgcn_fence(__ATOMIC_ACQUIRE, "workgroup");
        const char* src = reinterpret_cast<const char*>(ws) + ((size_t)w2 * (ACC * NT) + (size_t)tid * 4) * 4;
        typedef const __attribute__((address_space(1))) void* gptr_;
        typedef __attribute__((address_space(3))) void* lptr_;
        if (!(sk_abl & 2))
#pragma unroll
        for (int half = 0; half < 2; ++half) {
#pragma unroll
          for (int jq = 0; jq < 16; ++jq) {
            const int qg = half * 16 + jq;
            __builtin_amdgcn_global_load_lds((gptr_)(src + (size_t)(qg * NT) * 16), (lptr_)(smem_raw + (jq * NT + wave * 64) * 16), 16, 0, 17);
          }
          asm volatile("s_waitcnt vmcnt(0)" ::: "memory");
#pragma unroll
          for (int jq = 0; jq < 16; ++jq) {
            const int qg = half * 16 + jq;
            typedef float f32x4_ __attribute__((ext_vector_type(4)));
            const f32x4_ t4 = *reinterpret_cast<const f32x4_*>(smem_raw + (jq * NT + tid) * 16);
            const int blk = qg >> 2, r4 = qg & 3;
            const int mi = blk / (2 * NI), h = (blk / NI) & 1, ni = blk % NI;
#pragma unroll
            for (int e = 0; e < 4; ++e) acc[mi][h][ni][r4 * 4 + e] += t4[e];
          }
          asm volatile("s_waitcnt lgkmcnt(0)" ::: "memory");
        }
        __syncthreads();
        if (tid == 0) __hip_atomic_store(flags + w2, 0, __ATOMIC_RELAXED, __HIP_MEMORY_SCOPE_AGENT);
      }
    }
  }

  const ConvArgs& AT = *dv3_opaque_args<SK>(&args);
  const dv3_conv_desc& pt = AT.d;
  if (run_tail && (ABL != 3 || acc[0][0][0][0] + acc[1][1][1][7] == 1.2345e30f)) {
    if constexpr (F16) {
      constexpr float kInv = 1.0f / (float)(1 << (DV3_F16_WEIGHT_SHIFT + DV3_F16_ACT_SHIFT));
#pragma unroll
      for (int mi = 0; mi < MI; ++mi)
#pragma unroll
        for (int h = 0; h < 2; ++h)
#pragma unroll
          for (int ni = 0; ni < NI; ++ni)
#pragma unroll
            for (int r = 0; r < 16; ++r) acc[mi][h][ni][r] *= kInv;
    }
    int n0e = __builtin_amdgcn_readfirstlane(n0);
    asm volatile("" : "+s"(n0e));
    int bcol[NI], tcol[NI];
    bool okc[NI];
#pragma unroll
    for (int ni = 0; ni < NI; ++ni) {
      const int n = n0e + wn * (NI * 32) + ni * 32 + l31;
      okc[ni] = n < Ntot;
      bcol[ni] = n / T;
      tcol[ni] = n - bcol[ni] * T;
    }
    if constexpr (FG) {
      const int nw0 = n0e + wn * (NI * 32);
      if (dv3_wide_gate_ok(pt, AT.wide)) {
        float* wl = reinterpret_cast<float*>(smem_raw) + wave * (DV3_WIDE_LDS / 4);
#pragma unroll
        for (int mi = 0; mi < MI; ++mi) {
          const int row0 = wm * (MI * 32) + mi * 32;
          conv_epilogue_wide_block_gate<BM, BMH>(pt, acc[mi][0], mt, row0, 0, lane, nw0, Ntot, wl);
          conv_epilogue_wide_block_gate<BM, BMH>(pt, acc[mi][1], mt, row0, 1, lane, nw0, Ntot, wl);
        }
      } else {
        conv_epilogue_dgrad_gate<BM, BMH, NI>(pt, acc[0], mt, wm * (MI * 32), lhi, l31, bcol, tcol, okc, nw0 >> 5);
        conv_epilogue_dgrad_gate<BM, BMH, NI>(pt, acc[1], mt, wm * (MI * 32) + 32, lhi, l31, bcol, tcol, okc, nw0 >> 5);
      }
    } else
    if (ABL != 10 && dv3_wide_epilogue_ok(pt, AT.wide)) {
      float* wl = reinterpret_cast<float*>(smem_raw) + wave * (DV3_WIDE_LDS / 4);
      const int nw0 = n0e + wn * (NI * 32);
#pragma unroll
      for (int mi = 0; mi < MI; ++mi) {
        const int row0 = wm * (MI * 32) + mi * 32;
        conv_epilogue_wide_block<BM, BMH>(pt, acc[mi][0], mt, row0, 0, lane, nw0, Ntot, wl);
        conv_epilogue_wide_block<BM, BMH>(pt, acc[mi][1], mt, row0, 1, lane, nw0, Ntot, wl);
      }
    } else if (WIDE_GLU && dv3_wide_glu_ok(pt)) {
      constexpr int TA = ABL == 12 ? 12 : ABL == 13 ? 13 : 0;
      const int nw0 = n0e + wn * (NI * 32);
      conv_epilogue_glu_wide<BMH, NI, TA>(pt, acc[0], mt, wm * (MI * 32), lane, nw0, Ntot);
      conv_epilogue_glu_wide<BMH, NI, TA>(pt, acc[1], mt, wm * (MI * 32) + 32, lane, nw0, Ntot);
    } else {
      constexpr int TA = ABL == 12 ? 7 : ABL == 13 ? 8 : 0;
      bool interior = false;
      if constexpr (!SK)
        interior = TA == 0 && AT.fast_tail && gated && !pt.spk && pt.store_mode == DV3_STORE_BCT &&
                   mt * BMH + wm * (MI * 32) + MI * 32 <= pt.Cg && n0e + wn * (NI * 32) + NI * 32 <= Ntot;
      if (!SK && interior) {
        conv_epilogue_glu_interior<BMH, NI>(pt, acc[0], mt, wm * (MI * 32), lhi, bcol, tcol);
        conv_epilogue_glu_interior<BMH, NI>(pt, acc[1], mt, wm * (MI * 32) + 32, lhi, bcol, tcol);
      } else {
        conv_epilogue<BM, BMH, NI, TA, false>(pt, acc[0], gated, mt, wm * (MI * 32), lhi, bcol, tcol, okc);
        conv_epilogue<BM, BMH, NI, TA, false>(pt, acc[1], gated, mt, wm * (MI * 32) + 32, lhi, bcol, tcol, okc);
      }
    }
  }
  stamp();
  if constexpr (SK) {
    seg_u += c1 - c0;
    __syncthreads();
  }
  } while (SK && seg_u < seg_end);
}

#ifndef DV3_PP2_ISA_ONLY
template <bool MASK, bool F16, int ABL = 0, bool SK = false, int ORD = 0, bool PW = false, bool FG = false>
int launch_pp2(const ConvArgs& a, size_t lds, hipStream_t st) {
  if ((ORD & 4) != 0 && lds + 8 * 256 > 160 * 1024) return launch_pp2<MASK, F16, ABL, SK, (ORD & ~4), PW, FG>(a, lds, st);
  static bool attr_set = false;
  if (!attr_set) {
    hipError_t e = hipFuncSetAttribute((const void*)conv_gemm_pp2_kernel<MASK, F16, ABL, SK, ORD, PW, FG>,
                                       hipFuncAttributeMaxDynamicSharedMemorySize, 160 * 1024);
    if (e != hipSuccess) {
      dv3_set_error("conv_gemm_pp2: hipFuncSetAttribute: %s", hipGetErrorString(e));
      return DV3_ELAUNCH;
    }
    attr_set = true;
  }
  if ((ORD & 4) != 0) lds += 8 * 256;
  else if ((ORD & 64) != 0) lds += 32;
  hipLaunchKernelGGL((conv_gemm_pp2_kernel<MASK, F16, ABL, SK, ORD, PW, FG>), dim3(a.n_blocks), dim3(NT), lds, st, a);
  return dv3_check_launch("conv_gemm_pp2");
}

#endif
}

#ifndef DV3_PP2_ISA_ONLY
int dv3_pp2_read_stamps(void* dst, int64_t bytes) {
  if (bytes <= 0 || bytes > (int64_t)sizeof(unsigned long long) * 8 * PP2_STAMPS * 2) return DV3_EINVAL;
  return hipMemcpyFromSymbol(dst, HIP_SYMBOL(g_pp2_stamps), (size_t)bytes, 0, hipMemcpyDeviceToHost) == hipSuccess ? DV3_OK : DV3_ELAUNCH;
}
extern int g_x3_wide;
int g_pp2_ord = 0;
int g_pp2_ord_u = 81, g_pp2_ord_m = 81;
int g_pp2_fast_tail = 1;
int g_pp2_abl = 0;

int g_pp2_sk = 1;
int g_pp2_sk_overhead = 2;
int g_pp2_sk_gain = 80;
int g_pp2_sk_abl = 0;
static int pp2_cu_count() {
  static int n = 0;
  if (!n) {
    int dev = 0, v = 0;
    if (hipGetDevice(&dev) == hipSuccess && hipDeviceGetAttribute(&v, hipDeviceAttributeMultiprocessorCount, dev) == hipSuccess && v > 0) n = v;
    else n = 256;
  }
  return n;
}
int64_t dv3_pp2_sk_ws_bytes() { return (int64_t)pp2_cu_count() * (128 * NT * 4 + 64); }
extern "C" int dv3_conv_streamk_ws_bytes(void) { return (int)dv3_pp2_sk_ws_bytes(); }

int dv3_conv_gemm_pp2_dispatch(const dv3_conv_desc* d, hipStream_t st) {
  if (d->split_terms == 1 || !d->a_split) return 1;
  if (d->xmask && !d->xmask_c8) return 1;
  if (d->J != JT || (d->J - 1) * d->dil > HALO_MAX || (d->Cin & 31)) return 1;
  if (d->a_bs != 0 || (d->lda & 3) || d->Tin != d->Tout) return 1;
  const bool gated = d->mode == DV3_EPI_GLU || d->mode == DV3_EPI_HIGHWAY;
  const bool f16 = d->split_terms == DV3_SPLIT_F16X3;
  const int BNH = BN + (d->J - 1) * d->dil;
  const size_t lds = (size_t)(2 * 2 * KB * BM + 2 * 2 * KB * BNH) * 16;
  if (lds > 160 * 1024) return 1;
  ConvArgs a;
  a.d = *d;
  a.a_scalar = 0;
  a.wide = g_x3_wide;
  a.fast_tail = g_pp2_fast_tail;
  a.range_ctr = f16 ? dv3_range_ctr() : nullptr;
  a.kp = (d->Cin + 31) / 32 * 32;
  a.m_tiles = gated ? dv3_cdiv(d->Cg, BMH) : dv3_cdiv(d->M, BM);
  a.n_tiles = (int)dv3_cdiv64((int64_t)d->B * d->Tout, BN);
  const int64_t nb = (int64_t)a.m_tiles * a.n_tiles;
  DV3_REQUIRE(nb < (1ll << 31), "conv_gemm: grid too large");
  a.n_blocks = (int)nb;
  g_dv3_last_conv = (f16 ? 5000 : 3000) + 100 + 1;
  const bool mask = d->xmask_c8 != nullptr;
  if (d->x_pair || d->pg) {
    if (mask || f16) return 1;
    g_dv3_last_conv += (d->x_pair ? 5 : 0) + (d->pg ? 10 : 0);
    if (d->pg) return d->x_pair ? launch_pp2<false, false, 0, false, 81, true, true>(a, lds, st)
                                : launch_pp2<false, false, 0, false, 81, false, true>(a, lds, st);
    return launch_pp2<false, false, 0, false, 81, true>(a, lds, st);
  }
  {
    const int P = pp2_cu_count(), S = d->Cin / BKC;
    const int64_t units = nb * S;
    const int64_t dp = dv3_cdiv64(nb, P) * S, sk = dv3_cdiv64(units, P) + g_pp2_sk_overhead;
    const bool ws_ok = d->sk_ws && d->sk_ws_bytes >= dv3_pp2_sk_ws_bytes() && units < (1ll << 30);
    const bool dir_ok = d->mode != DV3_EPI_DGRAD || g_pp2_sk >= 2;
    const int q = P / 8;
    const bool grp_ok = (P % 8) == 0 && q > 0 && (q & (q - 1)) == 0 && nb >= 8;
    if (ws_ok && dir_ok && grp_ok && g_pp2_sk && (S & (S - 1)) == 0 && (a.m_tiles & (a.m_tiles - 1)) == 0 && units >= 2 * P && (g_pp2_sk == 2 || sk * 100 < dp * g_pp2_sk_gain)) {
      a.sk_abl = g_pp2_sk_abl;
      a.sk_units = (int)units;
      a.sk_tg = (int)(nb / 8);
      a.sk_tr = (int)(nb % 8);
      a.sk_qshift = __builtin_ctz((unsigned)q);
      const int64_t ub = (int64_t)(a.sk_tg + 1) * S, us = (int64_t)a.sk_tg * S;
      a.sk_base = (int)(ub / q);
      a.sk_rem = (int)(ub % q);
      a.sk_base2 = (int)(us / q);
      a.sk_rem2 = (int)(us % q);
      a.sk_shift = __builtin_ctz((unsigned)S);
      a.sk_mshift = __builtin_ctz((unsigned)a.m_tiles);
      a.n_blocks = P;
      a.sk_flags = reinterpret_cast<int*>(d->sk_ws);
      a.sk_ws = reinterpret_cast<float*>(reinterpret_cast<char*>(d->sk_ws) + (size_t)P * 64);
      g_dv3_last_conv += 1;
      const size_t lds_sk = lds;
      if (f16) return mask ? launch_pp2<true, true, 0, true>(a, lds_sk, st) : launch_pp2<false, true, 0, true>(a, lds_sk, st);
      return mask ? launch_pp2<true, false, 0, true>(a, lds_sk, st) : launch_pp2<false, false, 0, true>(a, lds_sk, st);
    }
  }
  {
    const int o = mask ? (f16 ? g_pp2_ord_m : 0) : g_pp2_ord_u;
#define DV3_PP2_ORD_SHIP(oo) \
    if (o == oo) { \
      if (f16) return mask ? launch_pp2<true, true, 0, false, oo>(a, lds, st) : launch_pp2<false, true, 0, false, oo>(a, lds, st); \
      return mask ? launch_pp2<true, false, 0, false, oo>(a, lds, st) : launch_pp2<false, false, 0, false, oo>(a, lds, st); \
    }
    DV3_PP2_ORD_SHIP(17) DV3_PP2_ORD_SHIP(81)
#undef DV3_PP2_ORD_SHIP
  }
#ifdef DV3_EXPERIMENTS
  if (g_pp2_ord && f16) {
    switch (g_pp2_ord) {
#define DV3_PP2_ORD_CASE(o) case o: return mask ? launch_pp2<true, true, 0, false, o>(a, lds, st) : launch_pp2<false, true, 0, false, o>(a, lds, st);
#define DV3_PP2_ORD_CASE_U(o) case o: if (!mask) return launch_pp2<false, true, 0, false, o>(a, lds, st); break;
      DV3_PP2_ORD_CASE_U(1) DV3_PP2_ORD_CASE_U(2) DV3_PP2_ORD_CASE_U(3) DV3_PP2_ORD_CASE_U(4) DV3_PP2_ORD_CASE_U(5) DV3_PP2_ORD_CASE_U(7)
      DV3_PP2_ORD_CASE_U(10) DV3_PP2_ORD_CASE_U(11) DV3_PP2_ORD_CASE_U(15)
      DV3_PP2_ORD_CASE(19) DV3_PP2_ORD_CASE(27) DV3_PP2_ORD_CASE(31) DV3_PP2_ORD_CASE(32) DV3_PP2_ORD_CASE(49) DV3_PP2_ORD_CASE(64) DV3_PP2_ORD_CASE(65)
#undef DV3_PP2_ORD_CASE_U
#undef DV3_PP2_ORD_CASE
    }
  }
  if (g_pp2_abl && !mask && f16) {
    switch (g_pp2_abl) {
      case 1: return launch_pp2<false, true, 1>(a, lds, st);
      case 2: return launch_pp2<false, true, 2>(a, lds, st);
      case 3: return launch_pp2<false, true, 3>(a, lds, st);
      case 4: return launch_pp2<false, true, 4>(a, lds, st);
      case 5: return launch_pp2<false, true, 5>(a, lds, st);
      case 6: return launch_pp2<false, true, 6>(a, lds, st);
      case 7: return launch_pp2<false, true, 7>(a, lds, st);
      case 8: return launch_pp2<false, true, 8>(a, lds, st);
      case 9: return launch_pp2<false, true, 9>(a, lds, st);
      case 10: return launch_pp2<false, true, 10>(a, lds, st);
      case 11: return launch_pp2<false, true, 11>(a, lds, st);
      case 12: return launch_pp2<false, true, 12>(a, lds, st);
      case 13: return launch_pp2<false, true, 13>(a, lds, st);
      case 14: return launch_pp2<false, true, 12, false, 32>(a, lds, st);
      case 15: return launch_pp2<false, true, 13, false, 32>(a, lds, st);
    }
  }
#endif
  if (f16) return mask ? launch_pp2<true, true>(a, lds, st) : launch_pp2<false, true>(a, lds, st);
  return mask ? launch_pp2<true, false>(a, lds, st) : launch_pp2<false, false>(a, lds, st);
}
#else
namespace {
template __global__ void conv_gemm_pp2_kernel<DV3_PP2_ISA_MASK, true, 0, false, DV3_PP2_ISA_ORD>(const ConvArgs);
}
#endif
```

Measured before the change: 3.827 million.

## Add straight-line two-segment stream-K variant of pp2 conv GEMM kernel

Moves the pp2 kernel body into an include file and adds an SL template flag. With SL, the stream-K loop over tile segments becomes at most two straight-line specialised segment bodies (a partial leading segment that stores partials, then the remaining one) instead of a generic do-while. The aim is to cut loop overhead and let the compiler specialise each segment's fixup and epilogue paths, including the interior GLU epilogue for stream-K. It is gated behind a new debug knob (g_pp2_sk_loop) and adds code size and more template instantiations.

```diff
diff --git a/deepvoice3_pytorch_amd/csrc/conv_gemm_bf16x3.hip b/deepvoice3_pytorch_amd/csrc/conv_gemm_bf16x3.hip
--- a/deepvoice3_pytorch_amd/csrc/conv_gemm_bf16x3.hip
+++ b/deepvoice3_pytorch_amd/csrc/conv_gemm_bf16x3.hip
@@ -802,7 +802,7 @@
 }
 
 int g_x3_pp2 = 128;
-extern int g_pp2_ord, g_pp2_ord_u, g_pp2_ord_m, g_pp2_abl, g_pp2_sk, g_pp2_sk_overhead, g_pp2_sk_gain, g_pp2_sk_abl, g_pp2_fast_tail;
+extern int g_pp2_ord, g_pp2_ord_u, g_pp2_ord_m, g_pp2_abl, g_pp2_sk, g_pp2_sk_overhead, g_pp2_sk_gain, g_pp2_sk_abl, g_pp2_sk_loop, g_pp2_fast_tail;
 int g_x3_pp2_sk_units = 8;
 int dv3_conv_gemm_pp2_dispatch(const dv3_conv_desc* d, hipStream_t st);
 int g_x3_wide = 1;
@@ -927,6 +927,7 @@
   if (what == 24) g_pp2_sk_gain = value;
   if (what == 25) g_x3_pp2_sk_units = value;
   if (what == 26) g_pp2_sk_abl = value;
+  if (what == 58) g_pp2_sk_loop = value;
   if (what == 27) g_x3_j1_flat = value;
   if (what == 43) g_x3_dp = value;
   if (what == 42) g_x3_rel8 = value;
diff --git a/deepvoice3_pytorch_amd/csrc/conv_gemm_pp2.hip b/deepvoice3_pytorch_amd/csrc/conv_gemm_pp2.hip
--- a/deepvoice3_pytorch_amd/csrc/conv_gemm_pp2.hip
+++ b/deepvoice3_pytorch_amd/csrc/conv_gemm_pp2.hip
@@ -52,8 +52,9 @@
 constexpr int PP2_STAMPS = 320;
 __device__ unsigned long long g_pp2_stamps[8 * PP2_STAMPS * 2];
 
-template <bool MASK, bool F16, int ABL = 0, bool SK = false, int ORD = 0, bool PW = false, bool FG = false>
+template <bool MASK, bool F16, int ABL = 0, bool SK = false, int ORD = 0, bool PW = false, bool FG = false, bool SL = false>
 __global__ __launch_bounds__(NT) void conv_gemm_pp2_kernel(const ConvArgs args) {
+  static_assert(!SL || SK, "straight-line segments: a stream-K form");
   static_assert(!PW || (!MASK && !F16 && !SK), "pair words: the unmasked bf16-pair tile-per-workgroup form");
   static_assert(!FG || (!MASK && !F16 && !SK), "fused gate backward: the unmasked bf16-pair tile-per-workgroup form");
   const dv3_conv_desc& p = args.d;
@@ -97,621 +98,28 @@
   constexpr bool WIDE_GLU = (ORD & 32) != 0;
   int tid_ = threadIdx.x;
   const int wave_s = __builtin_amdgcn_readfirstlane(tid_ >> 6);
+  if constexpr (SL) {
+    auto segment = [&](auto segc) __attribute__((always_inline)) {
+      constexpr int SEG = decltype(segc)::value;
+#include "conv_gemm_pp2_segment.inc"
+    };
+    if ((seg_u & (nchunks - 1)) != 0) segment(std::integral_constant<int, 1>{});
+    if (seg_u < seg_end) segment(std::integral_constant<int, 2>{});
+  } else {
   do {
-  const ConvArgs& A = *dv3_opaque_args<SK>(&args);
-  const dv3_conv_desc& p = A.d;
-  const int dil = p.dil;
-  const int BNH = BN + (J - 1) * dil;
-  const int xbuf = 2 * KB * BNH;
-  if constexpr (SK) {
-    int lane_;
-    asm volatile("v_mbcnt_lo_u32_b32 %0, -1, 0\n\tv_mbcnt_hi_u32_b32 %0, -1, %0" : "=v"(lane_));
-    tid_ = wave_s * 64 + lane_;
-  }
-  const int tid = tid_;
-  const int lane = tid & 63;
-  const int wave = __builtin_amdgcn_readfirstlane(tid >> 6);
-  const int wm = wave / WN, wn = wave % WN;
-  const int l31 = lane & 31, lhi = lane >> 5;
-  int tile_ = pid, c0_ = 0, c1_ = nchunks;
-  if constexpr (SK) {
-    tile_ = seg_u >> A.sk_shift;
-    c0_ = seg_u - tile_ * nchunks;
-    c1_ = min(nchunks, c0_ + (seg_end - seg_u));
-  }
-  const int tile = tile_, c0 = SK ? c0_ : 0, c1 = SK ? c1_ : nchunks;
-  const int mt = SK ? (tile & (A.m_tiles - 1)) : tile % A.m_tiles;
-  const int nt = SK ? (tile >> A.sk_mshift) : tile / A.m_tiles;
-  const int n0 = nt * BN;
-
-  const bool gated = (p.mode == DV3_EPI_GLU || p.mode == DV3_EPI_HIGHWAY);
-  int h0b, h1b;
-  if (gated) {
-    h0b = mt * BMH; h1b = p.a_half + mt * BMH;
-  } else {
-    h0b = mt * BM; h1b = mt * BM + BMH;
-  }
-
-  const int Cin = p.Cin, T = p.Tout, lda = p.lda, B = p.B;
-  const int Ntot = B * T;
-  const int k8_total = A.kp >> 3;
-  const bf16x8* __restrict__ Wh = reinterpret_cast<const bf16x8*>(p.a_split);
-  const int64_t plane = (int64_t)J * k8_total * lda;
-  const float xscale = F16 ? (float)(1 << DV3_F16_ACT_SHIFT) : 1.0f;
-  const float dscale = p.drop_scale * xscale;
-
-  uint32_t vbits = 0;
-#pragma unroll
-  for (int ni = 0; ni < NI; ++ni) {
-    const int n = n0 + wn * (NI * 32) + ni * 32 + l31;
-    const int bc = n / T, tc = n - bc * T;
-    for (int j = 0; j < J; ++j) {
-      const int ts = tc + j * dil - p.padL;
-      if (n < Ntot && ts >= 0 && ts < T) vbits |= 1u << (j * NI + ni);
-    }
-  }
-  uint32_t need = 0;
-  for (int j = 0; j < J; ++j) {
-    const uint32_t all = ((1u << NI) - 1u) << (j * NI);
-    if (!__all((vbits & all) == all)) need |= 1u << j;
-  }
-  need = __builtin_amdgcn_readfirstlane(need);
-
-  uint32_t xoff[XI];
-  const int n_items = KB * BNH;
-  const uint32_t x_rsb = (uint32_t)p.x_rs * 4u;
-  const uint32_t c8p = (uint32_t)((Cin + 31) / 32 * 4);
-#pragma unroll
-  for (int i = 0; i < XI; ++i) {
-    const int idx = tid + i * NT;
-    const int k8 = idx / BNH, q = idx - k8 * BNH;
-    const int f = n0 - p.padL + q;
-    int bf = 0, tf = 0;
-    if (idx < n_items && f >= 0 && f < Ntot) {
-      bf = f / T;
-      tf = f - bf * T;
-    }
-    const int xk8 = k8 < KB ? k8 * 8 : 0;
-    xoff[i] = ((uint32_t)bf * (uint32_t)p.x_bs + (uint32_t)tf) * 4u + (uint32_t)xk8 * x_rsb;
-  }
-  constexpr bool LEAN = (ORD & 2) != 0 && !SK;
-  uint32_t aoff_r[2] = {0u, 0u};
-  auto aoff_of = [&](int u) -> uint32_t {
-    if constexpr (LEAN) return aoff_r[u];
-    int t_ = tid;
-    asm volatile("" : "+v"(t_));
-    const int idx = t_ + u * NT;
-    const int col = idx % BM, k8 = idx / BM;
-    const bool hi_half = col >= BMH;
-    const int gcol = (hi_half ? h1b : h0b) + (col - (hi_half ? BMH : 0));
-    return (uint32_t)(k8 * lda + (gcol < lda ? gcol : 0)) * 16u;
-  };
-
-  if constexpr (LEAN) {
-#pragma unroll
-    for (int u = 0; u < 2; ++u) {
-      const int idx = tid + u * NT;
-      const int col = idx % BM, k8 = idx / BM;
-      const bool hi_half = col >= BMH;
-      const int gcol = (hi_half ? h1b : h0b) + (col - (hi_half ? BMH : 0));
-      aoff_r[u] = (uint32_t)(k8 * lda + (gcol < lda ? gcol : 0)) * 16u;
-    }
-  }
-
-  bf16x8 ra[2];
-  float rx[XI][8];
-  uint32_t rk[MASK ? XI : 1];
-
-  auto load_A_unit = [&](int chunk, int j, auto uc) {
-    constexpr int u = decltype(uc)::value;
-    const bf16x8* srch = Wh + (int64_t)(j * k8_total + chunk * KB) * lda;
-    const uint32_t ao = aoff_of(u);
-    ra[0] = pp2_ldg<bf16x8>(srch, ao);
-    ra[1] = pp2_ldg<bf16x8>(srch + plane, ao);
-  };
-  auto write_A_unit = [&](int buf, auto uc) {
-    constexpr int u = decltype(uc)::value;
-    bf16x8* dst = As + buf * (2 * KB * BM);
-    dst[tid + u * NT] = ra[0];
-    dst[KB * BM + tid + u * NT] = ra[1];
-  };
-  auto dma_A_unit = [&](int buf, int chunk, int j, auto uc) {
-    constexpr int u = decltype(uc)::value;
-    const bf16x8* srch = Wh + (int64_t)(j * k8_total + chunk * KB) * lda;
-    const uint32_t ao = aoff_of(u);
-    bf16x8* dst = As + buf * (2 * KB * BM) + u * NT + wave * 64;
-    typedef const __attribute__((address_space(1))) void* gptr;
-    typedef __attribute__((address_space(3))) void* lptr;
-    __builtin_amdgcn_global_load_lds((gptr)(reinterpret_cast<const char*>(srch) + ao), (lptr)dst, 16, 0, 0);
-    __builtin_amdgcn_global_load_lds((gptr)(reinterpret_cast<const char*>(srch + plane) + ao), (lptr)(dst + KB * BM), 16, 0, 0);
-  };
-  auto load_X_half = [&](int chunk, auto ic, auto hc) {
-    constexpr int i = decltype(ic)::value, h = decltype(hc)::value;
-    const char* xb = reinterpret_cast<const char*>(p.x) + (int64_t)(chunk * BKC) * x_rsb;
-    uint32_t rs = x_rsb;
-    asm volatile("" : "+s"(rs));
-#pragma unroll
-    for (int e = 4 * h; e < 4 * h + 4; ++e) {
-      uint32_t er = (uint32_t)e * rs;
-      if constexpr (SK) {
-        if (e == 0) { er = 0; asm volatile("" : "+s"(er)); }
-      }
-      rx[i][e] = pp2_ldg<float>(xb, xoff[i] + er);
-    }
-    if constexpr (MASK && h == 1) {
-      int t_ = tid;
-      asm volatile("" : "+v"(t_));
-      const int idx = t_ + i * NT;
-      const int k8 = idx / BNH, q = idx - k8 * BNH;
-      const int f = n0 - p.padL + q;
-      int bf = 0, tf = 0;
-      if (idx < n_items && f >= 0 && f < Ntot) {
-        bf = f / T;
-        tf = f - bf * T;
-      }
-      const uint32_t mo = ((uint32_t)bf * c8p + (uint32_t)(k8 < KB ? k8 : 0)) * (uint32_t)T + (uint32_t)tf;
-      rk[i] = (uint32_t)pp2_ldg<uint8_t>(p.xmask_c8 + (int64_t)chunk * 4 * T, mo);
-    }
-  };
-  auto write_X_item = [&](int buf, auto ic) {
-    constexpr int i = decltype(ic)::value;
-    bf16x8* dst = Xs + buf * xbuf;
-    const int idx = tid + i * NT;
-    float v[8];
-    uint32_t keep = MASK ? rk[i] : 0u;
-    if constexpr (MASK && SK) asm("" : "+v"(keep));
-#pragma unroll
-    for (int e = 0; e < 8; ++e) {
-      v[e] = rx[i][e];
-      if constexpr (MASK) v[e] *= ((keep >> e) & 1u) ? dscale : 0.f;
-      else if (F16) v[e] *= xscale;
-    }
-    bf16x8 hi, lo;
-    if constexpr (PW) {
-      uint32_t w[8];
-#pragma unroll
-      for (int e = 0; e < 8; ++e) w[e] = __float_as_uint(rx[i][e]);
-      dv3_pair_units(w, hi, lo);
-    } else if constexpr (F16 && LEAN) {
-      const float m0 = fmaxf(fmaxf(fabsf(v[0]), fabsf(v[1])), fabsf(v[2]));
-      const float m1 = fmaxf(fmaxf(fabsf(v[3]), fabsf(v[4])), fabsf(v[5]));
-      const float m = fmaxf(fmaxf(m0, m1), fmaxf(fabsf(v[6]), fabsf(v[7])));
-      const bool bad = !(m <= 65504.f);
-      if (__builtin_expect(__any(bad), 0)) {
-        dv3_note_range(A.range_ctr, dv3_split8_f16(v, hi, lo));
-      } else {
-        f16x8 h8, l8;
-#pragma unroll
-        for (int e = 0; e < 8; e += 2) {
-          const f32x2 f = {v[e], v[e + 1]};
-          typedef _Float16 f16x2_ __attribute__((ext_vector_type(2)));
-          const f16x2_ h = __builtin_convertvector(f, f16x2_);
-          h8[e] = h[0]; h8[e + 1] = h[1];
-          if constexpr ((ORD & 8) != 0) {
-            uint32_t l2 = 0u;
-            const uint32_t h2 = __builtin_bit_cast(uint32_t, h);
-            asm("v_fma_mixlo_f16 %0, %1, -1.0, %2 op_sel:[0,0,0] op_sel_hi:[1,0,0]" : "+v"(l2) : "v"(h2), "v"(v[e]));
-            asm("v_fma_mixhi_f16 %0, %1, -1.0, %2 op_sel:[1,0,0] op_sel_hi:[1,0,0]" : "+v"(l2) : "v"(h2), "v"(v[e + 1]));
-            const f16x2_ l = __builtin_bit_cast(f16x2_, l2);
-            l8[e] = l[0]; l8[e + 1] = l[1];
-          } else {
-            l8[e] = (_Float16)(v[e] - (float)h[0]);
-            l8[e + 1] = (_Float16)(v[e + 1] - (float)h[1]);
-          }
-        }
-        hi = __builtin_bit_cast(bf16x8, h8);
-        lo = __builtin_bit_cast(bf16x8, l8);
-      }
-    } else if constexpr (F16) dv3_note_range(A.range_ctr, dv3_split8_f16(v, hi, lo)); else pp2_split8(v, hi, lo);
-    if (idx < n_items) {
-      dst[idx] = hi;
-      dst[KB * BNH + idx] = lo;
-    }
-  };
-  uint32_t sbad = 0;
-  auto write_X_item_nb = [&](int buf, auto ic) {
-    constexpr int i = decltype(ic)::value;
-    bf16x8* dst = Xs + buf * xbuf;
-    const int idx = tid + i * NT;
-    float v[8];
-    const uint32_t keep = MASK ? rk[i] : 0u;
-#pragma unroll
-    for (int e = 0; e < 8; ++e) {
-      v[e] = rx[i][e];
-      if constexpr (MASK) {
-        v[e] *= ((keep >> e) & 1u) ? dscale : 0.f;
-        asm("" : "+v"(v[e]));
-      } else if (F16) v[e] *= xscale;
-    }
-    bf16x8 hi, lo;
-    if constexpr (PW) {
-      uint32_t w[8];
-#pragma unroll
-      for (int e = 0; e < 8; ++e) w[e] = __float_as_uint(rx[i][e]);
-      dv3_pair_units(w, hi, lo);
-    } else if constexpr (F16) {
-      const bool bad = dv3_split8_f16(v, hi, lo);
-      sbad += (uint32_t)__builtin_popcountll(__ballot(bad));
-    } else {
-      pp2_split8(v, hi, lo);
-    }
-    const int spare = 2 * xbuf - buf * xbuf;
-    const bool live = i < 2 || idx < n_items;
-    dst[live ? idx : spare] = hi;
-    dst[live ? KB * BNH + idx : spare + 1] = lo;
-  };
-  using U0 = std::integral_constant<int, 0>;
-  using U1 = std::integral_constant<int, 1>;
-  using U2 = std::integral_constant<int, 2>;
-  constexpr bool CVC = (ORD & 64) != 0 && !SK;
-  static_assert(XI == 3 && JT == 3, "three activation items per thread, one per tap's pair of k16 phases");
-
-  f32x16 acc[MI][2][NI];
-  float zero_ = 0.f;
-  if constexpr (SK) asm volatile("" : "+v"(zero_));
-#pragma unroll
-  for (int mi = 0; mi < MI; ++mi)
-#pragma unroll
-    for (int h = 0; h < 2; ++h)
-#pragma unroll
-      for (int ni = 0; ni < NI; ++ni)
-#pragma unroll
-        for (int r = 0; r < 16; ++r) acc[mi][h][ni][r] = zero_;
-
-  const int a_off = wm * (MI * 32) + l31;
-  const int x_off = wn * (NI * 32) + l31;
-
-  load_A_unit(c0, 0, U0{});
-  write_A_unit(0, U0{});
-  load_A_unit(c0, 0, U1{});
-  load_X_half(c0, U0{}, U0{}); load_X_half(c0, U0{}, U1{});
-  load_X_half(c0, U1{}, U0{}); load_X_half(c0, U1{}, U1{});
-  load_X_half(c0, U2{}, U0{}); load_X_half(c0, U2{}, U1{});
-  write_A_unit(0, U1{});
-  write_X_item(0, U0{});
-  write_X_item(0, U1{});
-  write_X_item(0, U2{});
-  __syncthreads();
-  {
-    const int cp = min(c0 + 1, c1 - 1);
-    if (!DMA_A) load_A_unit(c0, 1, U0{});
-    load_X_half(cp, U0{}, U0{});
-    load_X_half(cp, U0{}, U1{});
-    load_X_half(cp, U1{}, U0{}); load_X_half(cp, U1{}, U1{});
-    load_X_half(cp, U2{}, U0{});
-    if constexpr (!CVC) load_X_half(cp, U2{}, U1{});
-  }
-
-  const bool pf_on = (ORD & 4) != 0 && !SK && gated && p.r != nullptr;
-  const int late = wave >> 2;
-  stamp();
-  if (late) __syncthreads();
-  for (int c = c0; c < c1; ++c) {
-    const int cr = c - c0;
-    const bf16x8* XsH = Xs + (cr & 1) * xbuf;
-    const bf16x8* XsL = XsH + KB * BNH;
-    const int cx = min(c + 2, c1 - 1);
-    const bool last_chunk = c + 1 == c1;
-#pragma unroll
-    for (int q = 0; q < 2 * JT; ++q) {
-      constexpr int dummy = 0; (void)dummy;
-      const int j = q >> 1, s = q & 1;
-      const int cur = (cr * JT + j) & 1;
-      const bf16x8* AsH = As + cur * (2 * KB * BM);
-      const bf16x8* AsL = AsH + KB * BM;
-      const bool fix = (need >> j) & 1u;
-      stamp();
-      bf16x8 ah[MI][2], al[MI][2], bh[NI], bl[NI];
-      auto read_frags = [&](bool do_a, bool do_b) {
-        const int k8 = 2 * s + lhi;
-        if (do_a) {
-          const int ai = k8 * BM + a_off;
-#pragma unroll
-          for (int mi = 0; mi < MI; ++mi) {
-            ah[mi][0] = AsH[ai + mi * 32];
-            ah[mi][1] = AsH[ai + mi * 32 + BMH];
-            al[mi][0] = AsL[ai + mi * 32];
-            al[mi][1] = AsL[ai + mi * 32 + BMH];
-          }
-        }
-        if (do_b) {
-          const int xi = k8 * BNH + x_off + j * dil;
-#pragma unroll
-          for (int ni = 0; ni < NI; ++ni) {
-            bh[ni] = XsH[xi + ni * 32];
-            bl[ni] = XsL[xi + ni * 32];
-          }
-        }
-      };
-      auto fix_frags = [&]() {
-        const int k8 = 2 * s + lhi; (void)k8;
-        if (fix) {
-          const bf16x8 zero8 = {0, 0, 0, 0, 0, 0, 0, 0};
-#pragma unroll
-          for (int ni = 0; ni < NI; ++ni) {
-            const bool ok = (vbits >> (j * NI + ni)) & 1u;
-            bh[ni] = ok ? bh[ni] : zero8;
-            bl[ni] = ok ? bl[ni] : zero8;
-          }
-        }
-      };
-      if constexpr ((ORD & 1) != 0) {
-        read_frags(true, (ORD & 16) == 0);
-        __builtin_amdgcn_sched_barrier(0);
-      }
-      if (ABL != 2) {
-        int jn = j + 1, cn = c;
-        if (jn >= JT) { jn = 0; cn = c + 1; }
-        int j2 = jn + 1, c2 = cn;
-        if (j2 >= JT) { j2 = 0; c2 = cn + 1; }
-        if (cn >= c1) { cn = c; jn = j; }
-        if (c2 >= c1) { c2 = c; j2 = j; }
-        if constexpr (DMA_A) {
-          if (s == 0) {
-            dma_A_unit(cur ^ 1, cn, jn, U0{});
-            dma_A_unit(cur ^ 1, cn, jn, U1{});
-          }
-          (void)c2; (void)j2;
-        } else if (s == 0) {
-          if (ABL != 9) write_A_unit(cur ^ 1, U0{});
-          if (ABL != 7) load_A_unit(cn, jn, U1{});
-        } else {
-          if (ABL != 9) write_A_unit(cur ^ 1, U1{});
-          if (ABL != 7) load_A_unit(c2, j2, U0{});
-        }
-        constexpr bool WX = ABL != 8, LX = ABL != 6;
-        if constexpr (CVC) {
-          const int cx1 = min(c + 1, c1 - 1);
-          if (q == 0) load_X_half(cx1, U2{}, U1{});
-          if (q == 1) load_X_half(cx, U0{}, U0{});
-          if (q == 2) load_X_half(cx, U0{}, U1{});
-          if (q == 3) load_X_half(cx, U1{}, U0{});
-          if (q == 4) load_X_half(cx, U1{}, U1{});
-          if (q == 5) load_X_half(cx, U2{}, U0{});
-        } else {
-        if (q == 0) { if (WX) write_X_item((cr + 1) & 1, U0{}); if (LX) load_X_half(cx, U0{}, U0{}); }
-        if (q == 1) { if (LX) load_X_half(cx, U0{}, U1{}); }
-        if (q == 2) { if (WX) write_X_item((cr + 1) & 1, U1{}); if (LX) load_X_half(cx, U1{}, U0{}); }
-        if (q == 3) { if (LX) load_X_half(cx, U1{}, U1{}); }
-        if (q == 4) { if (WX) write_X_item((cr + 1) & 1, U2{}); if (LX) load_X_half(cx, U2{}, U0{}); }
-        if (q == 5) { if (LX) load_X_half(cx, U2{}, U1{}); }
-        }
-        if constexpr ((ORD & 4) != 0 && !SK) {
-          if ((q == 1 || q == 3) && last_chunk && pf_on) {
-            typedef const __attribute__((address_space(1))) void* gptr;
-            typedef __attribute__((address_space(3))) void* lptr;
-            unsigned char* strip = smem_raw + (size_t)(2 * 2 * KB * BM + 2 * xbuf) * 16 + wave * 256;
-            int t_ = tid;
-            asm volatile("" : "+v"(t_));
-            const int row = t_ >> 2, col = (t_ & 3) * 64 + (q >> 1) * 32;
-            const int ch = min(mt * BMH + row, p.Cg - 1);
-            const int n = min(n0 + col, Ntot - 1);
-            const int bb = n / T, tt = n - bb * T;
-            const uint32_t po = ((uint32_t)bb * (uint32_t)p.r_bs + (uint32_t)ch * (uint32_t)p.r_rs + (uint32_t)tt) * 4u;
-            __builtin_amdgcn_global_load_lds((gptr)(reinterpret_cast<const char*>(p.r) + po), (lptr)strip, 4, 0, 0);
-          }
-        }
-      }
-      __builtin_amdgcn_sched_barrier(0);
-      stamp();
-      if constexpr ((ORD & 1) == 0) read_frags(true, true);
-      else if constexpr ((ORD & 16) != 0) read_frags(false, true);
-      fix_frags();
-      if constexpr (ABL == 4) {
-        asm volatile("s_waitcnt lgkmcnt(0)" ::: "memory");
-        stamp();
-      }
-      __syncthreads();
-      if (ABL != 5) __builtin_amdgcn_sched_barrier(0);
-      stamp();
-      if (ABL != 1) {
-#pragma unroll
-        for (int mi = 0; mi < MI; ++mi)
-#pragma unroll
-          for (int ni = 0; ni < NI; ++ni) {
-            acc[mi][0][ni] = pp2_mma<F16>(al[mi][0], bh[ni], acc[mi][0][ni]);
-            acc[mi][1][ni] = pp2_mma<F16>(al[mi][1], bh[ni], acc[mi][1][ni]);
-          }
-#pragma unroll
-        for (int mi = 0; mi < MI; ++mi)
-#pragma unroll
-          for (int ni = 0; ni < NI; ++ni) {
-            acc[mi][0][ni] = pp2_mma<F16>(ah[mi][0], bl[ni], acc[mi][0][ni]);
-            acc[mi][1][ni] = pp2_mma<F16>(ah[mi][1], bl[ni], acc[mi][1][ni]);
-          }
-#pragma unroll
-        for (int mi = 0; mi < MI; ++mi)
-#pragma unroll
-          for (int ni = 0; ni < NI; ++ni) {
-            acc[mi][0][ni] = pp2_mma<F16>(ah[mi][0], bh[ni], acc[mi][0][ni]);
-            acc[mi][1][ni] = pp2_mma<F16>(ah[mi][1], bh[ni], acc[mi][1][ni]);
-          }
-      } else {
-#pragma unroll
-        for (int mi = 0; mi < MI; ++mi) asm volatile("" ::"v"(ah[mi][0]), "v"(ah[mi][1]), "v"(al[mi][0]), "v"(al[mi][1]));
-#pragma unroll
-        for (int ni = 0; ni < NI; ++ni) asm volatile("" ::"v"(bh[ni]), "v"(bl[ni]));
-      }
-      if constexpr (CVC) {
-        if (q == 0) write_X_item_nb((cr + 1) & 1, U0{});
-        if (q == 2) write_X_item_nb((cr + 1) & 1, U1{});
-        if (q == 4) write_X_item_nb((cr + 1) & 1, U2{});
-        if ((q & 1) == 0) {
-#pragma unroll
-          for (int m = 0; m < 22; ++m) {
-            __builtin_amdgcn_sched_group_barrier(0x008, 1, 0);
-            __builtin_amdgcn_sched_group_barrier(0x002, 3, 0);
-          }
-          __builtin_amdgcn_sched_group_barrier(0x008, 1, 0);
-          __builtin_amdgcn_sched_group_barrier(0x200, 1, 0);
-          __builtin_amdgcn_sched_group_barrier(0x008, 1, 0);
-          __builtin_amdgcn_sched_group_barrier(0x200, 1, 0);
-        }
-      }
-      stamp();
-      if (ABL != 5) __builtin_amdgcn_sched_barrier(0);
-      if (!(last_chunk && q == 2 * JT - 1) || !late) __syncthreads();
-    }
-  }
-  stamp();
-  if constexpr (CVC && F16) {
-    if (sbad != 0 && lane == 0 && A.range_ctr) atomicAdd(A.range_ctr, sbad);
-  }
-
-  bool run_tail = true;
-  if constexpr (SK) {
-    constexpr int ACC = MI * 2 * NI * 16;
-#ifdef DV3_EXPERIMENTS
-    const int sk_abl = A.sk_abl;
-#else
-    constexpr int sk_abl = 0;
-#endif
-    float* const ws = A.sk_ws;
-    int* const flags = A.sk_flags;
-    if (c0 != 0) {
-      char* dst = reinterpret_cast<char*>(ws) + ((size_t)pid * (ACC * NT) + (size_t)tid * 4) * 4;
-      if (!(sk_abl & 1))
-#pragma unroll
-      for (int mi = 0; mi < MI; ++mi)
-#pragma unroll
-        for (int h = 0; h < 2; ++h)
-#pragma unroll
-          for (int ni = 0; ni < NI; ++ni)
-#pragma unroll
-            for (int r4 = 0; r4 < 4; ++r4) {
-              typedef float f32x4_ __attribute__((ext_vector_type(4)));
-              const f32x4_ v4 = {acc[mi][h][ni][r4 * 4], acc[mi][h][ni][r4 * 4 + 1], acc[mi][h][ni][r4 * 4 + 2], acc[mi][h][ni][r4 * 4 + 3]};
-              const char* d4 = dst + (size_t)((((mi * 2 + h) * NI + ni) * 4 + r4) * NT) * 16;
-              asm volatile("global_store_dwordx4 %0, %1, off sc0 sc1" ::"v"(d4), "v"(v4) : "memory");
-            }
-      asm volatile("s_waitcnt vmcnt(0)" ::: "memory");
-      __builtin_amdgcn_fence(__ATOMIC_RELEASE, "workgroup");
-      __syncthreads();
-      if (tid == 0) __hip_atomic_store(flags + pid, 1, __ATOMIC_RELAXED, __HIP_MEMORY_SCOPE_AGENT);
-      run_tail = false;
-    } else if (c1 < nchunks) {
-      const int qm = (1 << A.sk_qshift) - 1;
-      for (int w2 = pid + 1; (w2 & qm) != 0; ++w2) {
-        const int s2 = sk_g0 + (w2 & qm) * sk_base + min(w2 & qm, sk_rem);
-        if (s2 >= (tile + 1) * nchunks) break;
-        if (tid == 0 && !(sk_abl & 4))
-          while (__hip_atomic_load(flags + w2, __ATOMIC_RELAXED, __HIP_MEMORY_SCOPE_AGENT) == 0) __builtin_amdgcn_s_sleep(8);
-        __syncthreads();
-        __builtin_amdgcn_fence(__ATOMIC_ACQUIRE, "workgroup");
-        const char* src = reinterpret_cast<const char*>(ws) + ((size_t)w2 * (ACC * NT) + (size_t)tid * 4) * 4;
-        typedef const __attribute__((address_space(1))) void* gptr_;
-        typedef __attribute__((address_space(3))) void* lptr_;
-        if (!(sk_abl & 2))
-#pragma unroll
-        for (int half = 0; half < 2; ++half) {
-#pragma unroll
-          for (int jq = 0; jq < 16; ++jq) {
-            const int qg = half * 16 + jq;
-            __builtin_amdgcn_global_load_lds((gptr_)(src + (size_t)(qg * NT) * 16), (lptr_)(smem_raw + (jq * NT + wave * 64) * 16), 16, 0, 17);
-          }
-          asm volatile("s_waitcnt vmcnt(0)" ::: "memory");
-#pragma unroll
-          for (int jq = 0; jq < 16; ++jq) {
-            const int qg = half * 16 + jq;
-            typedef float f32x4_ __attribute__((ext_vector_type(4)));
-            const f32x4_ t4 = *reinterpret_cast<const f32x4_*>(smem_raw + (jq * NT + tid) * 16);
-            const int blk = qg >> 2, r4 = qg & 3;
-            const int mi = blk / (2 * NI), h = (blk / NI) & 1, ni = blk % NI;
-#pragma unroll
-            for (int e = 0; e < 4; ++e) acc[mi][h][ni][r4 * 4 + e] += t4[e];
-          }
-          asm volatile("s_waitcnt lgkmcnt(0)" ::: "memory");
-        }
-        __syncthreads();
-        if (tid == 0) __hip_atomic_store(flags + w2, 0, __ATOMIC_RELAXED, __HIP_MEMORY_SCOPE_AGENT);
-      }
-    }
-  }
-
-  const ConvArgs& AT = *dv3_opaque_args<SK>(&args);
-  const dv3_conv_desc& pt = AT.d;
-  if (run_tail && (ABL != 3 || acc[0][0][0][0] + acc[1][1][1][7] == 1.2345e30f)) {
-    if constexpr (F16) {
-      constexpr float kInv = 1.0f / (float)(1 << (DV3_F16_WEIGHT_SHIFT + DV3_F16_ACT_SHIFT));
-#pragma unroll
-      for (int mi = 0; mi < MI; ++mi)
-#pragma unroll
-        for (int h = 0; h < 2; ++h)
-#pragma unroll
-          for (int ni = 0; ni < NI; ++ni)
-#pragma unroll
-            for (int r = 0; r < 16; ++r) acc[mi][h][ni][r] *= kInv;
-    }
-    int n0e = __builtin_amdgcn_readfirstlane(n0);
-    asm volatile("" : "+s"(n0e));
-    int bcol[NI], tcol[NI];
-    bool okc[NI];
-#pragma unroll
-    for (int ni = 0; ni < NI; ++ni) {
-      const int n = n0e + wn * (NI * 32) + ni * 32 + l31;
-      okc[ni] = n < Ntot;
-      bcol[ni] = n / T;
-      tcol[ni] = n - bcol[ni] * T;
-    }
-    if constexpr (FG) {
-      const int nw0 = n0e + wn * (NI * 32);
-      if (dv3_wide_gate_ok(pt, AT.wide)) {
-        float* wl = reinterpret_cast<float*>(smem_raw) + wave * (DV3_WIDE_LDS / 4);
-#pragma unroll
-        for (int mi = 0; mi < MI; ++mi) {
-          const int row0 = wm * (MI * 32) + mi * 32;
-          conv_epilogue_wide_block_gate<BM, BMH>(pt, acc[mi][0], mt, row0, 0, lane, nw0, Ntot, wl);
-          conv_epilogue_wide_block_gate<BM, BMH>(pt, acc[mi][1], mt, row0, 1, lane, nw0, Ntot, wl);
-        }
-      } else {
-        conv_epilogue_dgrad_gate<BM, BMH, NI>(pt, acc[0], mt, wm * (MI * 32), lhi, l31, bcol, tcol, okc, nw0 >> 5);
-        conv_epilogue_dgrad_gate<BM, BMH, NI>(pt, acc[1], mt, wm * (MI * 32) + 32, lhi, l31, bcol, tcol, okc, nw0 >> 5);
-      }
-    } else
-    if (ABL != 10 && dv3_wide_epilogue_ok(pt, AT.wide)) {
-      float* wl = reinterpret_cast<float*>(smem_raw) + wave * (DV3_WIDE_LDS / 4);
-      const int nw0 = n0e + wn * (NI * 32);
-#pragma unroll
-      for (int mi = 0; mi < MI; ++mi) {
-        const int row0 = wm * (MI * 32) + mi * 32;
-        conv_epilogue_wide_block<BM, BMH>(pt, acc[mi][0], mt, row0, 0, lane, nw0, Ntot, wl);
-        conv_epilogue_wide_block<BM, BMH>(pt, acc[mi][1], mt, row0, 1, lane, nw0, Ntot, wl);
-      }
-    } else if (WIDE_GLU && dv3_wide_glu_ok(pt)) {
-      constexpr int TA = ABL == 12 ? 12 : ABL == 13 ? 13 : 0;
-      const int nw0 = n0e + wn * (NI * 32);
-      conv_epilogue_glu_wide<BMH, NI, TA>(pt, acc[0], mt, wm * (MI * 32), lane, nw0, Ntot);
-      conv_epilogue_glu_wide<BMH, NI, TA>(pt, acc[1], mt, wm * (MI * 32) + 32, lane, nw0, Ntot);
-    } else {
-      constexpr int TA = ABL == 12 ? 7 : ABL == 13 ? 8 : 0;
-      bool interior = false;
-      if constexpr (!SK)
-        interior = TA == 0 && AT.fast_tail && gated && !pt.spk && pt.store_mode == DV3_STORE_BCT &&
-                   mt * BMH + wm * (MI * 32) + MI * 32 <= pt.Cg && n0e + wn * (NI * 32) + NI * 32 <= Ntot;
-      if (!SK && interior) {
-        conv_epilogue_glu_interior<BMH, NI>(pt, acc[0], mt, wm * (MI * 32), lhi, bcol, tcol);
-        conv_epilogue_glu_interior<BMH, NI>(pt, acc[1], mt, wm * (MI * 32) + 32, lhi, bcol, tcol);
-      } else {
-        conv_epilogue<BM, BMH, NI, TA, false>(pt, acc[0], gated, mt, wm * (MI * 32), lhi, bcol, tcol, okc);
-        conv_epilogue<BM, BMH, NI, TA, false>(pt, acc[1], gated, mt, wm * (MI * 32) + 32, lhi, bcol, tcol, okc);
-      }
-    }
-  }
-  stamp();
-  if constexpr (SK) {
-    seg_u += c1 - c0;
-    __syncthreads();
-  }
+  constexpr int SEG = 0;
+#include "conv_gemm_pp2_segment.inc"
   } while (SK && seg_u < seg_end);
+  }
 }
 
 #ifndef DV3_PP2_ISA_ONLY
-template <bool MASK, bool F16, int ABL = 0, bool SK = false, int ORD = 0, bool PW = false, bool FG = false>
+template <bool MASK, bool F16, int ABL = 0, bool SK = false, int ORD = 0, bool PW = false, bool FG = false, bool SL = false>
 int launch_pp2(const ConvArgs& a, size_t lds, hipStream_t st) {
-  if ((ORD & 4) != 0 && lds + 8 * 256 > 160 * 1024) return launch_pp2<MASK, F16, ABL, SK, (ORD & ~4), PW, FG>(a, lds, st);
+  if ((ORD & 4) != 0 && lds + 8 * 256 > 160 * 1024) return launch_pp2<MASK, F16, ABL, SK, (ORD & ~4), PW, FG, SL>(a, lds, st);
   static bool attr_set = false;
   if (!attr_set) {
-    hipError_t e = hipFuncSetAttribute((const void*)conv_gemm_pp2_kernel<MASK, F16, ABL, SK, ORD, PW, FG>,
+    hipError_t e = hipFuncSetAttribute((const void*)conv_gemm_pp2_kernel<MASK, F16, ABL, SK, ORD, PW, FG, SL>,
                                        hipFuncAttributeMaxDynamicSharedMemorySize, 160 * 1024);
     if (e != hipSuccess) {
       dv3_set_error("conv_gemm_pp2: hipFuncSetAttribute: %s", hipGetErrorString(e));
@@ -721,7 +129,7 @@
   }
   if ((ORD & 4) != 0) lds += 8 * 256;
   else if ((ORD & 64) != 0) lds += 32;
-  hipLaunchKernelGGL((conv_gemm_pp2_kernel<MASK, F16, ABL, SK, ORD, PW, FG>), dim3(a.n_blocks), dim3(NT), lds, st, a);
+  hipLaunchKernelGGL((conv_gemm_pp2_kernel<MASK, F16, ABL, SK, ORD, PW, FG, SL>), dim3(a.n_blocks), dim3(NT), lds, st, a);
   return dv3_check_launch("conv_gemm_pp2");
 }
 
@@ -743,6 +151,7 @@
 int g_pp2_sk_overhead = 2;
 int g_pp2_sk_gain = 80;
 int g_pp2_sk_abl = 0;
+int g_pp2_sk_loop = 0;
 static int pp2_cu_count() {
   static int n = 0;
   if (!n) {
@@ -812,6 +221,13 @@
       a.sk_ws = reinterpret_cast<float*>(reinterpret_cast<char*>(d->sk_ws) + (size_t)P * 64);
       g_dv3_last_conv += 1;
       const size_t lds_sk = lds;
+      const int share = max(a.sk_base + (a.sk_rem != 0), a.sk_base2 + (a.sk_rem2 != 0));
+      if (!g_pp2_sk_loop && share <= S) {
+        if (f16) return mask ? launch_pp2<true, true, 0, true, 81, false, false, true>(a, lds_sk, st)
+                             : launch_pp2<false, true, 0, true, 81, false, false, true>(a, lds_sk, st);
+        return mask ? launch_pp2<true, false, 0, true, 0, false, false, true>(a, lds_sk, st)
+                    : launch_pp2<false, false, 0, true, 0, false, false, true>(a, lds_sk, st);
+      }
       if (f16) return mask ? launch_pp2<true, true, 0, true>(a, lds_sk, st) : launch_pp2<false, true, 0, true>(a, lds_sk, st);
       return mask ? launch_pp2<true, false, 0, true>(a, lds_sk, st) : launch_pp2<false, false, 0, true>(a, lds_sk, st);
     }
diff --git a/deepvoice3_pytorch_amd/csrc/conv_gemm_pp2_segment.inc b/deepvoice3_pytorch_amd/csrc/conv_gemm_pp2_segment.inc
--- /dev/null
+++ b/deepvoice3_pytorch_amd/csrc/conv_gemm_pp2_segment.inc
@@ -0,0 +1,606 @@
+  const ConvArgs& A = *dv3_opaque_args<SK>(&args);
+  const dv3_conv_desc& p = A.d;
+  const int dil = p.dil;
+  const int BNH = BN + (J - 1) * dil;
+  const int xbuf = 2 * KB * BNH;
+  if constexpr (SK) {
+    int lane_;
+    asm volatile("v_mbcnt_lo_u32_b32 %0, -1, 0\n\tv_mbcnt_hi_u32_b32 %0, -1, %0" : "=v"(lane_));
+    tid_ = wave_s * 64 + lane_;
+  }
+  const int tid = tid_;
+  const int lane = tid & 63;
+  const int wave = __builtin_amdgcn_readfirstlane(tid >> 6);
+  const int wm = wave / WN, wn = wave % WN;
+  const int l31 = lane & 31, lhi = lane >> 5;
+  int tile_ = pid, c0_ = 0, c1_ = nchunks;
+  if constexpr (SK) {
+    tile_ = seg_u >> A.sk_shift;
+    c0_ = seg_u - tile_ * nchunks;
+    c1_ = min(nchunks, c0_ + (seg_end - seg_u));
+  }
+  const int tile = tile_, c0 = (SK && SEG != 2) ? c0_ : 0, c1 = SK ? c1_ : nchunks;
+  const int mt = SK ? (tile & (A.m_tiles - 1)) : tile % A.m_tiles;
+  const int nt = SK ? (tile >> A.sk_mshift) : tile / A.m_tiles;
+  const int n0 = nt * BN;
+
+  const bool gated = (p.mode == DV3_EPI_GLU || p.mode == DV3_EPI_HIGHWAY);
+  int h0b, h1b;
+  if (gated) {
+    h0b = mt * BMH; h1b = p.a_half + mt * BMH;
+  } else {
+    h0b = mt * BM; h1b = mt * BM + BMH;
+  }
+
+  const int Cin = p.Cin, T = p.Tout, lda = p.lda, B = p.B;
+  const int Ntot = B * T;
+  const int k8_total = A.kp >> 3;
+  const bf16x8* __restrict__ Wh = reinterpret_cast<const bf16x8*>(p.a_split);
+  const int64_t plane = (int64_t)J * k8_total * lda;
+  const float xscale = F16 ? (float)(1 << DV3_F16_ACT_SHIFT) : 1.0f;
+  const float dscale = p.drop_scale * xscale;
+
+  uint32_t vbits = 0;
+#pragma unroll
+  for (int ni = 0; ni < NI; ++ni) {
+    const int n = n0 + wn * (NI * 32) + ni * 32 + l31;
+    const int bc = n / T, tc = n - bc * T;
+    for (int j = 0; j < J; ++j) {
+      const int ts = tc + j * dil - p.padL;
+      if (n < Ntot && ts >= 0 && ts < T) vbits |= 1u << (j * NI + ni);
+    }
+  }
+  uint32_t need = 0;
+  for (int j = 0; j < J; ++j) {
+    const uint32_t all = ((1u << NI) - 1u) << (j * NI);
+    if (!__all((vbits & all) == all)) need |= 1u << j;
+  }
+  need = __builtin_amdgcn_readfirstlane(need);
+
+  uint32_t xoff[XI];
+  const int n_items = KB * BNH;
+  const uint32_t x_rsb = (uint32_t)p.x_rs * 4u;
+  const uint32_t c8p = (uint32_t)((Cin + 31) / 32 * 4);
+#pragma unroll
+  for (int i = 0; i < XI; ++i) {
+    const int idx = tid + i * NT;
+    const int k8 = idx / BNH, q = idx - k8 * BNH;
+    const int f = n0 - p.padL + q;
+    int bf = 0, tf = 0;
+    if (idx < n_items && f >= 0 && f < Ntot) {
+      bf = f / T;
+      tf = f - bf * T;
+    }
+    const int xk8 = k8 < KB ? k8 * 8 : 0;
+    xoff[i] = ((uint32_t)bf * (uint32_t)p.x_bs + (uint32_t)tf) * 4u + (uint32_t)xk8 * x_rsb;
+  }
+  constexpr bool LEAN = (ORD & 2) != 0 && !SK;
+  uint32_t aoff_r[2] = {0u, 0u};
+  auto aoff_of = [&](int u) -> uint32_t {
+    if constexpr (LEAN) return aoff_r[u];
+    int t_ = tid;
+    asm volatile("" : "+v"(t_));
+    const int idx = t_ + u * NT;
+    const int col = idx % BM, k8 = idx / BM;
+    const bool hi_half = col >= BMH;
+    const int gcol = (hi_half ? h1b : h0b) + (col - (hi_half ? BMH : 0));
+    return (uint32_t)(k8 * lda + (gcol < lda ? gcol : 0)) * 16u;
+  };
+
+  if constexpr (LEAN) {
+#pragma unroll
+    for (int u = 0; u < 2; ++u) {
+      const int idx = tid + u * NT;
+      const int col = idx % BM, k8 = idx / BM;
+      const bool hi_half = col >= BMH;
+      const int gcol = (hi_half ? h1b : h0b) + (col - (hi_half ? BMH : 0));
+      aoff_r[u] = (uint32_t)(k8 * lda + (gcol < lda ? gcol : 0)) * 16u;
+    }
+  }
+
+  bf16x8 ra[2];
+  float rx[XI][8];
+  uint32_t rk[MASK ? XI : 1];
+
+  auto load_A_unit = [&](int chunk, int j, auto uc) {
+    constexpr int u = decltype(uc)::value;
+    const bf16x8* srch = Wh + (int64_t)(j * k8_total + chunk * KB) * lda;
+    const uint32_t ao = aoff_of(u);
+    ra[0] = pp2_ldg<bf16x8>(srch, ao);
+    ra[1] = pp2_ldg<bf16x8>(srch + plane, ao);
+  };
+  auto write_A_unit = [&](int buf, auto uc) {
+    constexpr int u = decltype(uc)::value;
+    bf16x8* dst = As + buf * (2 * KB * BM);
+    dst[tid + u * NT] = ra[0];
+    dst[KB * BM + tid + u * NT] = ra[1];
+  };
+  auto dma_A_unit = [&](int buf, int chunk, int j, auto uc) {
+    constexpr int u = decltype(uc)::value;
+    const bf16x8* srch = Wh + (int64_t)(j * k8_total + chunk * KB) * lda;
+    const uint32_t ao = aoff_of(u);
+    bf16x8* dst = As + buf * (2 * KB * BM) + u * NT + wave * 64;
+    typedef const __attribute__((address_space(1))) void* gptr;
+    typedef __attribute__((address_space(3))) void* lptr;
+    __builtin_amdgcn_global_load_lds((gptr)(reinterpret_cast<const char*>(srch) + ao), (lptr)dst, 16, 0, 0);
+    __builtin_amdgcn_global_load_lds((gptr)(reinterpret_cast<const char*>(srch + plane) + ao), (lptr)(dst + KB * BM), 16, 0, 0);
+  };
+  auto load_X_half = [&](int chunk, auto ic, auto hc) {
+    constexpr int i = decltype(ic)::value, h = decltype(hc)::value;
+    const char* xb = reinterpret_cast<const char*>(p.x) + (int64_t)(chunk * BKC) * x_rsb;
+    uint32_t rs = x_rsb;
+    asm volatile("" : "+s"(rs));
+#pragma unroll
+    for (int e = 4 * h; e < 4 * h + 4; ++e) {
+      uint32_t er = (uint32_t)e * rs;
+      if constexpr (SK) {
+        if (e == 0) { er = 0; asm volatile("" : "+s"(er)); }
+      }
+      rx[i][e] = pp2_ldg<float>(xb, xoff[i] + er);
+    }
+    if constexpr (MASK && h == 1) {
+      int t_ = tid;
+      asm volatile("" : "+v"(t_));
+      const int idx = t_ + i * NT;
+      const int k8 = idx / BNH, q = idx - k8 * BNH;
+      const int f = n0 - p.padL + q;
+      int bf = 0, tf = 0;
+      if (idx < n_items && f >= 0 && f < Ntot) {
+        bf = f / T;
+        tf = f - bf * T;
+      }
+      const uint32_t mo = ((uint32_t)bf * c8p + (uint32_t)(k8 < KB ? k8 : 0)) * (uint32_t)T + (uint32_t)tf;
+      rk[i] = (uint32_t)pp2_ldg<uint8_t>(p.xmask_c8 + (int64_t)chunk * 4 * T, mo);
+    }
+  };
+  auto write_X_item = [&](int buf, auto ic) {
+    constexpr int i = decltype(ic)::value;
+    bf16x8* dst = Xs + buf * xbuf;
+    const int idx = tid + i * NT;
+    float v[8];
+    uint32_t keep = MASK ? rk[i] : 0u;
+    if constexpr (MASK && SK) asm("" : "+v"(keep));
+#pragma unroll
+    for (int e = 0; e < 8; ++e) {
+      v[e] = rx[i][e];
+      if constexpr (MASK) v[e] *= ((keep >> e) & 1u) ? dscale : 0.f;
+      else if (F16) v[e] *= xscale;
+    }
+    bf16x8 hi, lo;
+    if constexpr (PW) {
+      uint32_t w[8];
+#pragma unroll
+      for (int e = 0; e < 8; ++e) w[e] = __float_as_uint(rx[i][e]);
+      dv3_pair_units(w, hi, lo);
+    } else if constexpr (F16 && LEAN) {
+      const float m0 = fmaxf(fmaxf(fabsf(v[0]), fabsf(v[1])), fabsf(v[2]));
+      const float m1 = fmaxf(fmaxf(fabsf(v[3]), fabsf(v[4])), fabsf(v[5]));
+      const float m = fmaxf(fmaxf(m0, m1), fmaxf(fabsf(v[6]), fabsf(v[7])));
+      const bool bad = !(m <= 65504.f);
+      if (__builtin_expect(__any(bad), 0)) {
+        dv3_note_range(A.range_ctr, dv3_split8_f16(v, hi, lo));
+      } else {
+        f16x8 h8, l8;
+#pragma unroll
+        for (int e = 0; e < 8; e += 2) {
+          const f32x2 f = {v[e], v[e + 1]};
+          typedef _Float16 f16x2_ __attribute__((ext_vector_type(2)));
+          const f16x2_ h = __builtin_convertvector(f, f16x2_);
+          h8[e] = h[0]; h8[e + 1] = h[1];
+          if constexpr ((ORD & 8) != 0) {
+            uint32_t l2 = 0u;
+            const uint32_t h2 = __builtin_bit_cast(uint32_t, h);
+            asm("v_fma_mixlo_f16 %0, %1, -1.0, %2 op_sel:[0,0,0] op_sel_hi:[1,0,0]" : "+v"(l2) : "v"(h2), "v"(v[e]));
+            asm("v_fma_mixhi_f16 %0, %1, -1.0, %2 op_sel:[1,0,0] op_sel_hi:[1,0,0]" : "+v"(l2) : "v"(h2), "v"(v[e + 1]));
+            const f16x2_ l = __builtin_bit_cast(f16x2_, l2);
+            l8[e] = l[0]; l8[e + 1] = l[1];
+          } else {
+            l8[e] = (_Float16)(v[e] - (float)h[0]);
+            l8[e + 1] = (_Float16)(v[e + 1] - (float)h[1]);
+          }
+        }
+        hi = __builtin_bit_cast(bf16x8, h8);
+        lo = __builtin_bit_cast(bf16x8, l8);
+      }
+    } else if constexpr (F16) dv3_note_range(A.range_ctr, dv3_split8_f16(v, hi, lo)); else pp2_split8(v, hi, lo);
+    if (idx < n_items) {
+      dst[idx] = hi;
+      dst[KB * BNH + idx] = lo;
+    }
+  };
+  uint32_t sbad = 0;
+  auto write_X_item_nb = [&](int buf, auto ic) {
+    constexpr int i = decltype(ic)::value;
+    bf16x8* dst = Xs + buf * xbuf;
+    const int idx = tid + i * NT;
+    float v[8];
+    uint32_t keep = MASK ? rk[i] : 0u;
+    if constexpr (MASK && SK) asm("" : "+v"(keep));
+#pragma unroll
+    for (int e = 0; e < 8; ++e) {
+      v[e] = rx[i][e];
+      if constexpr (MASK) {
+        v[e] *= ((keep >> e) & 1u) ? dscale : 0.f;
+        asm("" : "+v"(v[e]));
+      } else if (F16) v[e] *= xscale;
+    }
+    bf16x8 hi, lo;
+    if constexpr (PW) {
+      uint32_t w[8];
+#pragma unroll
+      for (int e = 0; e < 8; ++e) w[e] = __float_as_uint(rx[i][e]);
+      dv3_pair_units(w, hi, lo);
+    } else if constexpr (F16) {
+      const bool bad = dv3_split8_f16(v, hi, lo);
+      sbad += (uint32_t)__builtin_popcountll(__ballot(bad));
+    } else {
+      pp2_split8(v, hi, lo);
+    }
+    const int spare = 2 * xbuf - buf * xbuf;
+    const bool live = i < 2 || idx < n_items;
+    dst[live ? idx : spare] = hi;
+    dst[live ? KB * BNH + idx : spare + 1] = lo;
+  };
+  using U0 = std::integral_constant<int, 0>;
+  using U1 = std::integral_constant<int, 1>;
+  using U2 = std::integral_constant<int, 2>;
+  constexpr bool CVC = (ORD & 64) != 0 && (!SK || SL);
+  static_assert(XI == 3 && JT == 3, "three activation items per thread, one per tap's pair of k16 phases");
+
+  f32x16 acc[MI][2][NI];
+  float zero_ = 0.f;
+  if constexpr (SK) asm volatile("" : "+v"(zero_));
+#pragma unroll
+  for (int mi = 0; mi < MI; ++mi)
+#pragma unroll
+    for (int h = 0; h < 2; ++h)
+#pragma unroll
+      for (int ni = 0; ni < NI; ++ni)
+#pragma unroll
+        for (int r = 0; r < 16; ++r) acc[mi][h][ni][r] = zero_;
+
+  const int a_off = wm * (MI * 32) + l31;
+  const int x_off = wn * (NI * 32) + l31;
+
+  load_A_unit(c0, 0, U0{});
+  write_A_unit(0, U0{});
+  load_A_unit(c0, 0, U1{});
+  load_X_half(c0, U0{}, U0{}); load_X_half(c0, U0{}, U1{});
+  load_X_half(c0, U1{}, U0{}); load_X_half(c0, U1{}, U1{});
+  load_X_half(c0, U2{}, U0{}); load_X_half(c0, U2{}, U1{});
+  write_A_unit(0, U1{});
+  write_X_item(0, U0{});
+  write_X_item(0, U1{});
+  write_X_item(0, U2{});
+  __syncthreads();
+  {
+    const int cp = min(c0 + 1, c1 - 1);
+    if (!DMA_A) load_A_unit(c0, 1, U0{});
+    load_X_half(cp, U0{}, U0{});
+    load_X_half(cp, U0{}, U1{});
+    load_X_half(cp, U1{}, U0{}); load_X_half(cp, U1{}, U1{});
+    load_X_half(cp, U2{}, U0{});
+    if constexpr (!CVC) load_X_half(cp, U2{}, U1{});
+  }
+
+  const bool pf_on = (ORD & 4) != 0 && !SK && gated && p.r != nullptr;
+  const int late = wave >> 2;
+  stamp();
+  if (late) __syncthreads();
+  for (int c = c0; c < c1; ++c) {
+    const int cr = c - c0;
+    const bf16x8* XsH = Xs + (cr & 1) * xbuf;
+    const bf16x8* XsL = XsH + KB * BNH;
+    const int cx = min(c + 2, c1 - 1);
+    const bool last_chunk = c + 1 == c1;
+#pragma unroll
+    for (int q = 0; q < 2 * JT; ++q) {
+      constexpr int dummy = 0; (void)dummy;
+      const int j = q >> 1, s = q & 1;
+      const int cur = (cr * JT + j) & 1;
+      const bf16x8* AsH = As + cur * (2 * KB * BM);
+      const bf16x8* AsL = AsH + KB * BM;
+      const bool fix = (need >> j) & 1u;
+      stamp();
+      bf16x8 ah[MI][2], al[MI][2], bh[NI], bl[NI];
+      auto read_frags = [&](bool do_a, bool do_b) {
+        const int k8 = 2 * s + lhi;
+        if (do_a) {
+          const int ai = k8 * BM + a_off;
+#pragma unroll
+          for (int mi = 0; mi < MI; ++mi) {
+            ah[mi][0] = AsH[ai + mi * 32];
+            ah[mi][1] = AsH[ai + mi * 32 + BMH];
+            al[mi][0] = AsL[ai + mi * 32];
+            al[mi][1] = AsL[ai + mi * 32 + BMH];
+          }
+        }
+        if (do_b) {
+          const int xi = k8 * BNH + x_off + j * dil;
+#pragma unroll
+          for (int ni = 0; ni < NI; ++ni) {
+            bh[ni] = XsH[xi + ni * 32];
+            bl[ni] = XsL[xi + ni * 32];
+          }
+        }
+      };
+      auto fix_frags = [&]() {
+        const int k8 = 2 * s + lhi; (void)k8;
+        if (fix) {
+          const bf16x8 zero8 = {0, 0, 0, 0, 0, 0, 0, 0};
+#pragma unroll
+          for (int ni = 0; ni < NI; ++ni) {
+            const bool ok = (vbits >> (j * NI + ni)) & 1u;
+            bh[ni] = ok ? bh[ni] : zero8;
+            bl[ni] = ok ? bl[ni] : zero8;
+          }
+        }
+      };
+      if constexpr ((ORD & 1) != 0) {
+        read_frags(true, (ORD & 16) == 0);
+        __builtin_amdgcn_sched_barrier(0);
+      }
+      if (ABL != 2) {
+        int jn = j + 1, cn = c;
+        if (jn >= JT) { jn = 0; cn = c + 1; }
+        int j2 = jn + 1, c2 = cn;
+        if (j2 >= JT) { j2 = 0; c2 = cn + 1; }
+        if (cn >= c1) { cn = c; jn = j; }
+        if (c2 >= c1) { c2 = c; j2 = j; }
+        if constexpr (DMA_A) {
+          if (s == 0) {
+            dma_A_unit(cur ^ 1, cn, jn, U0{});
+            dma_A_unit(cur ^ 1, cn, jn, U1{});
+          }
+          (void)c2; (void)j2;
+        } else if (s == 0) {
+          if (ABL != 9) write_A_unit(cur ^ 1, U0{});
+          if (ABL != 7) load_A_unit(cn, jn, U1{});
+        } else {
+          if (ABL != 9) write_A_unit(cur ^ 1, U1{});
+          if (ABL != 7) load_A_unit(c2, j2, U0{});
+        }
+        constexpr bool WX = ABL != 8, LX = ABL != 6;
+        if constexpr (CVC) {
+          const int cx1 = min(c + 1, c1 - 1);
+          if (q == 0) load_X_half(cx1, U2{}, U1{});
+          if (q == 1) load_X_half(cx, U0{}, U0{});
+          if (q == 2) load_X_half(cx, U0{}, U1{});
+          if (q == 3) load_X_half(cx, U1{}, U0{});
+          if (q == 4) load_X_half(cx, U1{}, U1{});
+          if (q == 5) load_X_half(cx, U2{}, U0{});
+        } else {
+        if (q == 0) { if (WX) write_X_item((cr + 1) & 1, U0{}); if (LX) load_X_half(cx, U0{}, U0{}); }
+        if (q == 1) { if (LX) load_X_half(cx, U0{}, U1{}); }
+        if (q == 2) { if (WX) write_X_item((cr + 1) & 1, U1{}); if (LX) load_X_half(cx, U1{}, U0{}); }
+        if (q == 3) { if (LX) load_X_half(cx, U1{}, U1{}); }
+        if (q == 4) { if (WX) write_X_item((cr + 1) & 1, U2{}); if (LX) load_X_half(cx, U2{}, U0{}); }
+        if (q == 5) { if (LX) load_X_half(cx, U2{}, U1{}); }
+        }
+        if constexpr ((ORD & 4) != 0 && !SK) {
+          if ((q == 1 || q == 3) && last_chunk && pf_on) {
+            typedef const __attribute__((address_space(1))) void* gptr;
+            typedef __attribute__((address_space(3))) void* lptr;
+            unsigned char* strip = smem_raw + (size_t)(2 * 2 * KB * BM + 2 * xbuf) * 16 + wave * 256;
+            int t_ = tid;
+            asm volatile("" : "+v"(t_));
+            const int row = t_ >> 2, col = (t_ & 3) * 64 + (q >> 1) * 32;
+            const int ch = min(mt * BMH + row, p.Cg - 1);
+            const int n = min(n0 + col, Ntot - 1);
+            const int bb = n / T, tt = n - bb * T;
+            const uint32_t po = ((uint32_t)bb * (uint32_t)p.r_bs + (uint32_t)ch * (uint32_t)p.r_rs + (uint32_t)tt) * 4u;
+            __builtin_amdgcn_global_load_lds((gptr)(reinterpret_cast<const char*>(p.r) + po), (lptr)strip, 4, 0, 0);
+          }
+        }
+      }
+      __builtin_amdgcn_sched_barrier(0);
+      stamp();
+      if constexpr ((ORD & 1) == 0) read_frags(true, true);
+      else if constexpr ((ORD & 16) != 0) read_frags(false, true);
+      fix_frags();
+      if constexpr (ABL == 4) {
+        asm volatile("s_waitcnt lgkmcnt(0)" ::: "memory");
+        stamp();
+      }
+      __syncthreads();
+      if (ABL != 5) __builtin_amdgcn_sched_barrier(0);
+      stamp();
+      if (ABL != 1) {
+#pragma unroll
+        for (int mi = 0; mi < MI; ++mi)
+#pragma unroll
+          for (int ni = 0; ni < NI; ++ni) {
+            acc[mi][0][ni] = pp2_mma<F16>(al[mi][0], bh[ni], acc[mi][0][ni]);
+            acc[mi][1][ni] = pp2_mma<F16>(al[mi][1], bh[ni], acc[mi][1][ni]);
+          }
+#pragma unroll
+        for (int mi = 0; mi < MI; ++mi)
+#pragma unroll
+          for (int ni = 0; ni < NI; ++ni) {
+            acc[mi][0][ni] = pp2_mma<F16>(ah[mi][0], bl[ni], acc[mi][0][ni]);
+            acc[mi][1][ni] = pp2_mma<F16>(ah[mi][1], bl[ni], acc[mi][1][ni]);
+          }
+#pragma unroll
+        for (int mi = 0; mi < MI; ++mi)
+#pragma unroll
+          for (int ni = 0; ni < NI; ++ni) {
+            acc[mi][0][ni] = pp2_mma<F16>(ah[mi][0], bh[ni], acc[mi][0][ni]);
+            acc[mi][1][ni] = pp2_mma<F16>(ah[mi][1], bh[ni], acc[mi][1][ni]);
+          }
+      } else {
+#pragma unroll
+        for (int mi = 0; mi < MI; ++mi) asm volatile("" ::"v"(ah[mi][0]), "v"(ah[mi][1]), "v"(al[mi][0]), "v"(al[mi][1]));
+#pragma unroll
+        for (int ni = 0; ni < NI; ++ni) asm volatile("" ::"v"(bh[ni]), "v"(bl[ni]));
+      }
+      if constexpr (CVC) {
+        if (q == 0) write_X_item_nb((cr + 1) & 1, U0{});
+        if (q == 2) write_X_item_nb((cr + 1) & 1, U1{});
+        if (q == 4) write_X_item_nb((cr + 1) & 1, U2{});
+        if ((q & 1) == 0) {
+#pragma unroll
+          for (int m = 0; m < 22; ++m) {
+            __builtin_amdgcn_sched_group_barrier(0x008, 1, 0);
+            __builtin_amdgcn_sched_group_barrier(0x002, 3, 0);
+          }
+          __builtin_amdgcn_sched_group_barrier(0x008, 1, 0);
+          __builtin_amdgcn_sched_group_barrier(0x200, 1, 0);
+          __builtin_amdgcn_sched_group_barrier(0x008, 1, 0);
+          __builtin_amdgcn_sched_group_barrier(0x200, 1, 0);
+        }
+      }
+      stamp();
+      if (ABL != 5) __builtin_amdgcn_sched_barrier(0);
+      if (!(last_chunk && q == 2 * JT - 1) || !late) __syncthreads();
+    }
+  }
+  stamp();
+  if constexpr (CVC && F16) {
+    if (sbad != 0 && lane == 0 && A.range_ctr) atomicAdd(A.range_ctr, sbad);
+  }
+
+  bool run_tail = true;
+  if constexpr (SK) {
+    constexpr int ACC = MI * 2 * NI * 16;
+#ifdef DV3_EXPERIMENTS
+    const int sk_abl = A.sk_abl;
+#else
+    constexpr int sk_abl = 0;
+#endif
+    float* const ws = A.sk_ws;
+    int* const flags = A.sk_flags;
+    if (SEG == 1 || (SEG == 0 && c0 != 0)) {
+      char* dst = reinterpret_cast<char*>(ws) + ((size_t)pid * (ACC * NT) + (size_t)tid * 4) * 4;
+      if (!(sk_abl & 1))
+#pragma unroll
+      for (int mi = 0; mi < MI; ++mi)
+#pragma unroll
+        for (int h = 0; h < 2; ++h)
+#pragma unroll
+          for (int ni = 0; ni < NI; ++ni)
+#pragma unroll
+            for (int r4 = 0; r4 < 4; ++r4) {
+              typedef float f32x4_ __attribute__((ext_vector_type(4)));
+              const f32x4_ v4 = {acc[mi][h][ni][r4 * 4], acc[mi][h][ni][r4 * 4 + 1], acc[mi][h][ni][r4 * 4 + 2], acc[mi][h][ni][r4 * 4 + 3]};
+              const char* d4 = dst + (size_t)((((mi * 2 + h) * NI + ni) * 4 + r4) * NT) * 16;
+              asm volatile("global_store_dwordx4 %0, %1, off sc0 sc1" ::"v"(d4), "v"(v4) : "memory");
+            }
+      asm volatile("s_waitcnt vmcnt(0)" ::: "memory");
+      __builtin_amdgcn_fence(__ATOMIC_RELEASE, "workgroup");
+      __syncthreads();
+      if (tid == 0) __hip_atomic_store(flags + pid, 1, __ATOMIC_RELAXED, __HIP_MEMORY_SCOPE_AGENT);
+      run_tail = false;
+    } else if (SEG != 1 && c1 < nchunks) {
+      const int qm = (1 << A.sk_qshift) - 1;
+      for (int w2 = pid + 1; (w2 & qm) != 0; ++w2) {
+        const int s2 = sk_g0 + (w2 & qm) * sk_base + min(w2 & qm, sk_rem);
+        if (s2 >= (tile + 1) * nchunks) break;
+        if (tid == 0 && !(sk_abl & 4))
+          while (__hip_atomic_load(flags + w2, __ATOMIC_RELAXED, __HIP_MEMORY_SCOPE_AGENT) == 0) __builtin_amdgcn_s_sleep(8);
+        __syncthreads();
+        __builtin_amdgcn_fence(__ATOMIC_ACQUIRE, "workgroup");
+        const char* src = reinterpret_cast<const char*>(ws) + ((size_t)w2 * (ACC * NT) + (size_t)tid * 4) * 4;
+        typedef const __attribute__((address_space(1))) void* gptr_;
+        typedef __attribute__((address_space(3))) void* lptr_;
+        if (!(sk_abl & 2))
+#pragma unroll
+        for (int half = 0; half < 2; ++half) {
+#pragma unroll
+          for (int jq = 0; jq < 16; ++jq) {
+            const int qg = half * 16 + jq;
+            __builtin_amdgcn_global_load_lds((gptr_)(src + (size_t)(qg * NT) * 16), (lptr_)(smem_raw + (jq * NT + wave * 64) * 16), 16, 0, 17);
+          }
+          asm volatile("s_waitcnt vmcnt(0)" ::: "memory");
+#pragma unroll
+          for (int jq = 0; jq < 16; ++jq) {
+            const int qg = half * 16 + jq;
+            typedef float f32x4_ __attribute__((ext_vector_type(4)));
+            const f32x4_ t4 = *reinterpret_cast<const f32x4_*>(smem_raw + (jq * NT + tid) * 16);
+            const int blk = qg >> 2, r4 = qg & 3;
+            const int mi = blk / (2 * NI), h = (blk / NI) & 1, ni = blk % NI;
+#pragma unroll
+            for (int e = 0; e < 4; ++e) acc[mi][h][ni][r4 * 4 + e] += t4[e];
+          }
+          asm volatile("s_waitcnt lgkmcnt(0)" ::: "memory");
+        }
+        __syncthreads();
+        if (tid == 0) __hip_atomic_store(flags + w2, 0, __ATOMIC_RELAXED, __HIP_MEMORY_SCOPE_AGENT);
+      }
+    }
+  }
+
+  const ConvArgs& AT = *dv3_opaque_args<SK>(&args);
+  const dv3_conv_desc& pt = AT.d;
+  if (run_tail && (ABL != 3 || acc[0][0][0][0] + acc[1][1][1][7] == 1.2345e30f)) {
+    if constexpr (F16) {
+      constexpr float kInv = 1.0f / (float)(1 << (DV3_F16_WEIGHT_SHIFT + DV3_F16_ACT_SHIFT));
+#pragma unroll
+      for (int mi = 0; mi < MI; ++mi)
+#pragma unroll
+        for (int h = 0; h < 2; ++h)
+#pragma unroll
+          for (int ni = 0; ni < NI; ++ni)
+#pragma unroll
+            for (int r = 0; r < 16; ++r) acc[mi][h][ni][r] *= kInv;
+    }
+    int n0e = __builtin_amdgcn_readfirstlane(n0);
+    asm volatile("" : "+s"(n0e));
+    int bcol[NI], tcol[NI];
+    bool okc[NI];
+#pragma unroll
+    for (int ni = 0; ni < NI; ++ni) {
+      const int n = n0e + wn * (NI * 32) + ni * 32 + l31;
+      okc[ni] = n < Ntot;
+      bcol[ni] = n / T;
+      tcol[ni] = n - bcol[ni] * T;
+    }
+    if constexpr (FG) {
+      const int nw0 = n0e + wn * (NI * 32);
+      if (dv3_wide_gate_ok(pt, AT.wide)) {
+        float* wl = reinterpret_cast<float*>(smem_raw) + wave * (DV3_WIDE_LDS / 4);
+#pragma unroll
+        for (int mi = 0; mi < MI; ++mi) {
+          const int row0 = wm * (MI * 32) + mi * 32;
+          conv_epilogue_wide_block_gate<BM, BMH>(pt, acc[mi][0], mt, row0, 0, lane, nw0, Ntot, wl);
+          conv_epilogue_wide_block_gate<BM, BMH>(pt, acc[mi][1], mt, row0, 1, lane, nw0, Ntot, wl);
+        }
+      } else {
+        conv_epilogue_dgrad_gate<BM, BMH, NI>(pt, acc[0], mt, wm * (MI * 32), lhi, l31, bcol, tcol, okc, nw0 >> 5);
+        conv_epilogue_dgrad_gate<BM, BMH, NI>(pt, acc[1], mt, wm * (MI * 32) + 32, lhi, l31, bcol, tcol, okc, nw0 >> 5);
+      }
+    } else
+    if (ABL != 10 && dv3_wide_epilogue_ok(pt, AT.wide)) {
+      float* wl = reinterpret_cast<float*>(smem_raw) + wave * (DV3_WIDE_LDS / 4);
+      const int nw0 = n0e + wn * (NI * 32);
+#pragma unroll
+      for (int mi = 0; mi < MI; ++mi) {
+        const int row0 = wm * (MI * 32) + mi * 32;
+        conv_epilogue_wide_block<BM, BMH>(pt, acc[mi][0], mt, row0, 0, lane, nw0, Ntot, wl);
+        conv_epilogue_wide_block<BM, BMH>(pt, acc[mi][1], mt, row0, 1, lane, nw0, Ntot, wl);
+      }
+    } else if (WIDE_GLU && dv3_wide_glu_ok(pt)) {
+      constexpr int TA = ABL == 12 ? 12 : ABL == 13 ? 13 : 0;
+      const int nw0 = n0e + wn * (NI * 32);
+      conv_epilogue_glu_wide<BMH, NI, TA>(pt, acc[0], mt, wm * (MI * 32), lane, nw0, Ntot);
+      conv_epilogue_glu_wide<BMH, NI, TA>(pt, acc[1], mt, wm * (MI * 32) + 32, lane, nw0, Ntot);
+    } else {
+      constexpr int TA = ABL == 12 ? 7 : ABL == 13 ? 8 : 0;
+      constexpr bool HAS_INTERIOR = !SK || SL;
+      bool interior = false;
+      if constexpr (HAS_INTERIOR)
+        interior = TA == 0 && AT.fast_tail && gated && !pt.spk && pt.store_mode == DV3_STORE_BCT &&
+                   mt * BMH + wm * (MI * 32) + MI * 32 <= pt.Cg && n0e + wn * (NI * 32) + NI * 32 <= Ntot;
+      if (HAS_INTERIOR && interior) {
+        conv_epilogue_glu_interior<BMH, NI>(pt, acc[0], mt, wm * (MI * 32), lhi, bcol, tcol);
+        conv_epilogue_glu_interior<BMH, NI>(pt, acc[1], mt, wm * (MI * 32) + 32, lhi, bcol, tcol);
+      } else {
+        conv_epilogue<BM, BMH, NI, TA, false>(pt, acc[0], gated, mt, wm * (MI * 32), lhi, bcol, tcol, okc);
+        conv_epilogue<BM, BMH, NI, TA, false>(pt, acc[1], gated, mt, wm * (MI * 32) + 32, lhi, bcol, tcol, okc);
+      }
+    }
+  }
+  stamp();
+  if constexpr (SK) {
+    seg_u += c1 - c0;
+    __syncthreads();
+  }
```

After: 3.869 million (median of 6 runs). 1.1% higher.
